# niclasborlin/dbat

Measured on AMD Instinct MI355X. Metric: LM iterations/sec, higher is better.
Workload: dtype f64

## Files before the change

dbat_amd/_hip.py:

```python
from __future__ import annotations

import ctypes as C
import os
import sys

import numpy as np

_HERE = os.path.dirname(os.path.abspath(__file__))
LIB_PATH = os.path.join(_HERE, 'libdbat_hip.so')
if os.environ.get('DBAT_AMD_LIB') == 'prof':
    LIB_PATH = os.path.join(_HERE, 'libdbat_hip_prof.so')
elif os.environ.get('DBAT_AMD_LIB', '').endswith('.so'):
    LIB_PATH = os.environ['DBAT_AMD_LIB']
if LIB_PATH != os.path.join(_HERE, 'libdbat_hip.so'):
    sys.stderr.write('[dbat_amd] DBAT_AMD_LIB: loading %s instead of the product library\n' % LIB_PATH)

ABI_VERSION = 5
DAMP = {'none': 0, 'gm': 0, 'gna': 1, 'lm': 2, 'lmp': 3}

OK, EINVAL, EUNSUPPORTED, EDEVICE, ENOMEM = 0, -101, -102, -103, -104


class DbatHipUnavailable(RuntimeError):
    pass
# ... 25 lines not shown
        ('device', C.c_int32), ('shard_rank', C.c_int32), ('shard_count', C.c_int32),
    ]


class Options(C.Structure):
    _fields_ = [
        ('damping', C.c_int32), ('max_iter', C.c_int32), ('conv_tol', C.c_double),
        ('abs_term', C.c_int32), ('singular_test', C.c_int32), ('store_trace', C.c_int32),
        ('mu', C.c_double), ('alpha_min', C.c_double), ('lambda0', C.c_double),
        ('lambda_min', C.c_double), ('rho_bad', C.c_double), ('rho_good', C.c_double),
        ('delta0', C.c_double),
        ('term_fun', C.c_void_p), ('term_user', C.c_void_p), ('veto_fun', C.c_void_p), ('veto_user', C.c_void_p),
        ('trace_fun', C.c_void_p), ('trace_user', C.c_void_p),
    ]


TERM_FN = C.CFUNCTYPE(C.c_int32, C.c_void_p, _dp, _dp, C.c_int64)
VETO_FN = C.CFUNCTYPE(C.c_int32, C.c_void_p, _dp, C.c_int64)
TRACE_FN = C.CFUNCTYPE(None, C.c_void_p, C.c_int32, C.c_int32, C.c_double, C.c_double, C.c_int32, C.c_double)


def trace_text(damping, n, res, damp, step, rho):
    from fractions import Fraction
    if damping == DAMP['gna']:
        if damp != damp:
            return 'Gauss-Newton-Armijo: iteration %d, residual norm=%.2g' % (n, res)
        return 'Gauss-Newton-Armijo: iteration %d, residual norm=%.2g, last alpha=%s' % (n, res, Fraction(damp).limit_denominator(1 << 40))
    if damping == DAMP['lm']:
        if damp != damp:
            return 'Levenberg-Marquardt: iteration %d, residual norm=%.2g' % (n, res)
        return 'Levenberg-Marquardt: iteration %d, residual norm=%.2g, lambda=%.2g' % (n, res, damp)
    if damping == DAMP['lmp']:
        return 'Levenberg-Marquardt-Powell: iteration %d, residual norm=%.2g, delta=%.2g, step=%s, rho=%.1f' % (
            n, res, damp, ('GN', 'IP', 'CP')[step] if 0 <= step < 3 else '?', rho)
    return 'Gauss-Markov: iteration %d, residual norm=%.2g' % (n, res)


class Result(C.Structure):
    _fields_ = [
        ('code', C.c_int32), ('iters', C.c_int32), ('n_res', C.c_int32), ('n_damp', C.c_int32),
        ('n_trace', C.c_int32), ('sigma0', C.c_double), ('time_s', C.c_double),
        ('n_residual_evals', C.c_int32), ('n_linearizations', C.c_int32), ('n_solves', C.c_int32),
        ('n_trace_only', C.c_int32), ('stage_s', C.c_double * 5),
    ]


LOSS = {'huber': 0, 'cauchy': 1}
SCALE = {'apriori': 0, 'mad': 1}
ROBUST_MAX_OUTER = 64


class RobustOptions(C.Structure):
    _fields_ = [
        ('loss', C.c_int32), ('k', C.c_double), ('scale', C.c_int32), ('max_outer', C.c_int32),
        ('weight_tol', C.c_double),
    ]


class PairOptions(C.Structure):
    _fields_ = [('max_iter', C.c_int32), ('conv_tol', C.c_double), ('min_angle', C.c_double)]


class RobustResult(C.Structure):
    _fields_ = [
        ('outer', C.c_int32), ('converged', C.c_int32), ('inner_iters', C.c_int32 * ROBUST_MAX_OUTER),
        ('scale', C.c_double * ROBUST_MAX_OUTER), ('max_change', C.c_double), ('reweight_s', C.c_double),
    ]


ALLREDUCE_FN = C.CFUNCTYPE(C.c_int, C.c_void_p, C.c_void_p, C.c_int64, C.c_void_p)

class DepthStats(C.Structure):
    _fields_ = [('n_behind', C.c_int64), ('min_depth', C.c_double), ('argmin_column', C.c_int64)]


class VetoStats(C.Structure):
    _fields_ = [('tested', C.c_int64), ('rejected', C.c_int64), ('n_behind', C.c_int64), ('min_depth', C.c_double)]


_H = C.c_void_p
SYMBOLS = {
    'dbat_hip_last_error': (C.c_char_p, []),
    'dbat_hip_abi_version': (C.c_int, []),
    'dbat_hip_default_options': (C.c_int, [C.c_int32, C.POINTER(Options)]),
    'dbat_hip_plan': (C.c_int, [C.POINTER(Problem)] + [C.POINTER(C.c_int64)] * 7),
    'dbat_hip_plan_structural_rank_ok': (C.c_int, [C.POINTER(Problem), C.POINTER(C.c_int32)]),
    'dbat_hip_plan_point_owner': (C.c_int, [C.POINTER(Problem), _ip]),
    'dbat_hip_plan_serialize': (C.c_int, [C.POINTER(Problem), _dp]),
    'dbat_hip_plan_layout_stats': (C.c_int, [C.POINTER(Problem), C.POINTER(C.c_int64)]),
    'dbat_hip_plan_domain_map': (C.c_int, [C.POINTER(Problem), _ip, C.POINTER(C.c_int32)]),
    'dbat_hip_create': (C.c_int, [C.POINTER(Problem), C.POINTER(_H)]),
    'dbat_hip_destroy': (None, [_H]),
    'dbat_hip_num_params': (C.c_int64, [_H]),
    'dbat_hip_num_residuals': (C.c_int64, [_H]),
    'dbat_hip_serialize': (C.c_int, [_H, _dp]),
    'dbat_hip_deserialize': (C.c_int, [_H, _dp, _dp, _dp, _dp]),
    'dbat_hip_structural_rank_ok': (C.c_int, [_H, C.POINTER(C.c_int32)]),
    'dbat_hip_residual': (C.c_int, [_H, _dp, _dp, _dp]),
    'dbat_hip_jacobian_blocks': (C.c_int, [_H, _dp, _dp, _dp, _dp]),
    'dbat_hip_jacobian_sample': (C.c_int, [_H, _dp, C.c_int64, C.POINTER(C.c_int64), _dp, _dp, _dp, _dp]),
    'dbat_hip_linearize_solve': (C.c_int, [_H, _dp, C.c_double, C.c_int32, _dp, _dp]),
    'dbat_hip_jacobian_csc': (C.c_int, [_H, _dp, C.c_int32, C.POINTER(C.c_int64), C.POINTER(C.c_int64), C.POINTER(C.c_int64), _dp]),
    'dbat_hip_gradient': (C.c_int, [_H, _dp]),
    'dbat_hip_colnorms': (C.c_int, [_H, _dp]),
    'dbat_hip_jtimes_sqnorm': (C.c_int, [_H, _dp, _dp]),
    'dbat_hip_jtimes': (C.c_int, [_H, _dp, _dp]),
    'dbat_hip_solve': (C.c_int, [_H, C.POINTER(Options), _dp, C.POINTER(Result), _dp, _dp, _dp, _dp]),
    'dbat_hip_final_residuals': (C.c_int, [_H, _dp, _dp]),
    'dbat_hip_comm_unique_id': (C.c_int, [_bp]),
    'dbat_hip_comm_init': (C.c_int, [_H, _bp]),
    'dbat_hip_comm_allreduce_host': (C.c_int, [_H, _dp, C.c_int64, C.c_int32]),
    'dbat_hip_set_deterministic': (C.c_int, [_H, C.c_int32]),
    'dbat_hip_set_allreduce': (C.c_int, [_H, ALLREDUCE_FN, C.c_void_p]),
    'dbat_hip_owned_mask': (C.c_int, [_H, _bp]),
    'dbat_hip_forwintersect': (C.c_int, [_H, _dp, _bp, _dp]),
    'dbat_hip_resect': (C.c_int, [C.c_int32, C.c_int32, C.POINTER(C.c_int64), _dp, _dp, C.POINTER(C.c_int64), _ip, _dp, _dp]),
    'dbat_hip_rigidalign': (C.c_int, [C.c_int32, C.c_int64, _dp, _dp, _bp, C.c_int32, _dp, _dp, _dp]),
    'dbat_hip_multixform': (C.c_int, [C.c_int32, _dp, C.c_int64, C.c_int32, _dp, C.c_int64, _dp, _bp]),
    'dbat_hip_essmat5': (C.c_int, [C.c_int32, C.c_int32, C.POINTER(C.c_int64), _dp, _dp, _dp, _ip]),
    'dbat_hip_relorient': (C.c_int, [C.c_int32, C.c_int32, C.POINTER(C.c_int64), _dp, _dp, C.POINTER(C.c_int64), _ip, _dp,
                                     C.c_int32, _dp, _dp, _ip, _bp, _bp, _dp]),
    'dbat_hip_default_pair_options': (C.c_int, [C.POINTER(PairOptions)]),
    'dbat_hip_pairadjust': (C.c_int, [C.c_int32, C.c_int32, C.POINTER(C.c_int64), _dp, _dp, _bp, _dp, _dp, C.c_int32,
                                      C.POINTER(PairOptions), _dp, _dp, _bp, _dp, _ip, _dp, _dp]),
    'dbat_hip_bench_step': (C.c_int, [_H, C.c_double, C.c_int32, _dp]),
    'dbat_hip_structure_key': (C.c_int, [C.POINTER(Problem), C.POINTER(C.c_uint64)]),
    'dbat_hip_handle_key': (C.c_int, [_H, C.POINTER(C.c_uint64)]),
    'dbat_hip_set_values': (C.c_int, [_H, C.POINTER(Problem)]),
    'dbat_hip_set_x': (C.c_int, [_H, _dp]),
    'dbat_hip_info': (C.c_int, [_H, C.POINTER(C.c_int64)]),
    'dbat_hip_build_kernel_name': (C.c_int, [_H, C.c_char_p, C.c_int32]),
    'dbat_hip_chol_stats': (C.c_int, [_H, C.POINTER(C.c_int64)]),
    'dbat_hip_posterior_cov': (C.c_int, [_H, _dp, C.c_double, _dp, _dp, _dp, _dp]),
    'dbat_hip_redundancy': (C.c_int, [_H, _dp, _dp, _dp]),
    'dbat_hip_ray_angles': (C.c_int, [_H, _dp, _dp, _dp, _ip, _ip]),
    'dbat_hip_debug_ray_angles_host': (C.c_int, [C.POINTER(Problem), _dp, _dp]),
    'dbat_hip_point_depths': (C.c_int, [_H, _dp, C.c_double, _dp, _dp, C.POINTER(DepthStats)]),
    'dbat_hip_set_chirality': (C.c_int, [_H, C.c_int32, C.c_double]),
    'dbat_hip_chirality_stats': (C.c_int, [_H, C.POINTER(VetoStats)]),
    'dbat_hip_coverage': (C.c_int, [_H, _dp, _dp, _dp, _lp, _dp, _lp, _lp]),
    'dbat_hip_residual_stats': (C.c_int, [_H, _dp, _lp, _dp, _lp, _dp, _dp, _dp, _lp]),
    'dbat_hip_quality_hull_cap': (C.c_int32, []),
    'dbat_hip_debug_coverage_host': (C.c_int, [C.POINTER(Problem), _dp, _dp, _dp, _lp, _dp, _lp, _lp]),
    'dbat_hip_default_robust_options': (C.c_int, [C.c_int32, C.POINTER(RobustOptions)]),
    'dbat_hip_robust_weights': (C.c_int, [_H, _dp, C.POINTER(RobustOptions), _dp, _dp, _dp]),
    'dbat_hip_set_obs_weights': (C.c_int, [_H, _dp]),
    'dbat_hip_solve_robust': (C.c_int, [_H, C.POINTER(Options), C.POINTER(RobustOptions), _dp, C.POINTER(Result),
                                        _dp, _dp, _dp, _dp, C.POINTER(RobustResult), _dp]),
}
DEBUG_SYMBOLS = {
    'dbat_hip_debug_plan_digest': (C.c_int, [C.POINTER(Problem), C.POINTER(C.c_uint64), C.c_int32, C.c_char_p, C.c_int32]),
    'dbat_hip_debug_heavy_plan_selftest': (C.c_int, [C.POINTER(Problem), _dp]),
    'dbat_hip_debug_batch_stats': (C.c_int, [C.POINTER(Problem), C.POINTER(C.c_int64)]),
    'dbat_hip_debug_model_eval_host': (C.c_int, [C.c_int32, C.c_int32, C.c_int32, _dp, _dp, C.c_double,
                                                 _dp, _dp, _dp, _dp, _dp, _dp]),
    'dbat_hip_debug_ray_angles_ms': (C.c_int, [_H, _dp, C.POINTER(C.c_int64)]),
    'dbat_hip_debug_quality_ms': (C.c_int, [_H, _dp]),
    'dbat_hip_debug_point_depths_ms': (C.c_int, [_H, _dp]),
    'dbat_hip_debug_chirality_pass_ms': (C.c_int, [_H, _dp, C.c_int32, _dp]),
    'dbat_hip_debug_align_ms': (C.c_int, [_dp]),
    'dbat_hip_debug_align_timing': (C.c_int, [C.c_int32]),
    'dbat_hip_debug_relorient_ms': (C.c_int, [_dp]),
    'dbat_hip_debug_relorient_timing': (C.c_int, [C.c_int32]),
    'dbat_hip_debug_pairadjust_ms': (C.c_int, [_dp]),
    'dbat_hip_debug_pairadjust_timing': (C.c_int, [C.c_int32]),
}

_lib = None


def load():
    global _lib
    if _lib is not None:
        return _lib
    if not os.path.exists(LIB_PATH):
        raise DbatHipUnavailable(
            '%s not built: run `python -c "import __graft_entry__ as g; g.build()"` or '
            '`make -C dbat_amd/csrc` (needs hipcc).  There is no CPU fallback.' % LIB_PATH)
    try:
        try:
            import torch
        except Exception:
            pass
        lib = C.CDLL(LIB_PATH)
    except OSError as e:
        raise DbatHipUnavailable('cannot load %s: %s' % (LIB_PATH, e)) from e
    for name, (res, args) in {**SYMBOLS, **DEBUG_SYMBOLS}.items():
        try:
            fn = getattr(lib, name)
        except AttributeError as e:
            raise DbatHipUnavailable('%s does not export %s' % (LIB_PATH, name)) from e
        fn.restype = res
        fn.argtypes = args
    if lib.dbat_hip_abi_version() != ABI_VERSION:
        raise DbatHipUnavailable('ABI version mismatch')
    _lib = lib
    return lib


UNIQUE_ID_BYTES = 128


def comm_unique_id():
    buf = (C.c_uint8 * UNIQUE_ID_BYTES)()
    check(load().dbat_hip_comm_unique_id(buf))
    return bytes(buf)


def last_error():
    return load().dbat_hip_last_error().decode('utf-8', 'replace')


def check(rc):
    if rc != 0:
        raise DbatHipError(rc, last_error())


def dptr(a):
    return a.ctypes.data_as(_dp) if a is not None else None


def _flat(a, dtype):
    a = np.asarray(a)
    if a.dtype != dtype:
        a = a.astype(dtype)
    if a.ndim <= 1:
        return np.ascontiguousarray(a)
    if a.flags.f_contiguous:
        return a.reshape(-1, order='F')
    return a.flatten('F')


def _f64(a):
    return _flat(a, np.float64)


def _u8(a):
    a = np.asarray(a)
    if a.dtype != np.bool_:
        a = a.astype(bool)
    return _flat(a, np.bool_).view(np.uint8)


def _i32(a):
    return _flat(a, np.int32)


def problem_from_struct(s, device=0, shard_rank=0, shard_count=1):
    nc, npnt, no = s.EO.val.shape[1], s.OP.val.shape[1], s.IP.val.shape[1]
    dm = np.unique(s.IO.model.distModel)
    if dm.size != 1:
        raise ValueError('Mixed lens distortion models not implemented.')
    model = int(dm[0])
    if model == 1:
        if np.any(np.asarray(s.IO.val)[3:5] != 0) or np.any(np.asarray(s.bundle.est.IO)[3:5]):
            raise ValueError('lens distortion model 1 has no aspect/skew')
        model = 2
    if npnt >= 2 ** 31 or nc >= 2 ** 31:
        raise ValueError('too many points/images for int32 indices')
    keep = dict(
        ip_cam=_i32(s.IP.cam), ip_pt=_i32(s.IP.pt), ip_val=_f64(s.IP.val), ip_std=_f64(s.IP.std),
        IO_val=_f64(s.IO.val), px_size=_f64(s.IO.sensor.pxSize), EO_val=_f64(s.EO.val[:6]),
        OP_val=_f64(s.OP.val),
        est_IO=_u8(s.bundle.est.IO), est_EO=_u8(s.bundle.est.EO[:6]), est_OP=_u8(s.bundle.est.OP),
        IO_block=_i32(s.IO.struct.block), EO_block=_i32(s.EO.struct.block[:6]),
    )
    for nm in ('IO', 'EO', 'OP'):
        pr = getattr(s.prior, nm)
        rows = slice(0, 6) if nm == 'EO' else slice(None)
        use = np.asarray(pr.use)[rows]
        keep['prior_%s_use' % nm] = _u8(use)
        if use.any():
            keep['prior_%s_val' % nm] = _f64(np.nan_to_num(np.asarray(pr.val, float)[rows]))
            keep['prior_%s_std' % nm] = _f64(np.nan_to_num(np.asarray(pr.std, float)[rows], nan=1.0))
        else:
            keep['prior_%s_val' % nm] = _f64(np.asarray(pr.val, float)[rows])
            keep['prior_%s_std' % nm] = _f64(np.asarray(pr.std, float)[rows])
    p = Problem()
    p.abi_version = ABI_VERSION
    p.n_images, p.n_points, p.n_obs = nc, npnt, no
    p.dist_model, p.nK, p.nP = model, int(s.IO.model.nK), int(s.IO.model.nP)
    for k, v in keep.items():
        ptr_t = dict(Problem._fields_)[k]
        setattr(p, k, v.ctypes.data_as(ptr_t))
    p.device, p.shard_rank, p.shard_count = int(device), int(shard_rank), int(shard_count)
    return p, keep


class Handle:

    def __init__(self, s, device=0, shard_rank=0, shard_count=1, _problem=None):
        self.lib = load()
        self.prob, self._keep = _problem if _problem is not None else problem_from_struct(s, device, shard_rank, shard_count)
        h = _H()
        check(self.lib.dbat_hip_create(C.byref(self.prob), C.byref(h)))
        self.h = h
        self.n = int(self.lib.dbat_hip_num_params(h))
        self.m = int(self.lib.dbat_hip_num_residuals(h))
        self._cb = None

    def close(self):
        if getattr(self, 'h', None):
            self.lib.dbat_hip_destroy(self.h)
            self.h = None

    __del__ = close
# ... 493 lines not shown
    return dict(E=E[:9 * n].reshape(n, 9), P2=P2[:12 * n].reshape(n, 4, 3).transpose(0, 2, 1), stats=st[:8 * n].reshape(n, 8),
                inlier=inl[:total].astype(bool), in_front=fr[:total].astype(bool), X=X[:3 * total].reshape(3, total, order='F'))


def cams_from_e(e, x1, x2, front_dir, device=0):
    lib = load()
    x1, x2 = np.asarray(x1, float), np.asarray(x2, float)
    if x1.ndim != 2 or x1.shape[0] != 2 or x1.shape != x2.shape:
        raise ValueError('camsfrome: the points must be 2-by-n')
    n = x1.shape[1]
    ps = np.array([0, n], np.int64)
    a, b, E, t2 = _f64(x1), _f64(x2), np.ascontiguousarray(np.asarray(e, float).reshape(9)).copy(), np.ones(1)
    P2, st = np.zeros(12), np.zeros(8, np.int32)
    inl, fr, X = np.zeros(max(n, 1), np.uint8), np.zeros(max(n, 1), np.uint8), np.zeros(3 * max(n, 1))
    check(lib.dbat_hip_relorient(int(device), 1, ps.ctypes.data_as(C.POINTER(C.c_int64)), dptr(a), dptr(b), None, None, dptr(t2),
                                 int(front_dir), dptr(E), dptr(P2), st.ctypes.data_as(_ip), inl.ctypes.data_as(_bp),
                                 fr.ctypes.data_as(_bp), dptr(X)))
    return dict(P2=P2.reshape(4, 3).T.copy(), X=X[:3 * n].reshape(3, n, order='F'), in_front=fr[:n].astype(bool), sp=st[4:8].copy())


def relorient_timing(on=True):
    check(load().dbat_hip_debug_relorient_timing(int(bool(on))))


def relorient_ms():
    ms = np.zeros(3)
    check(load().dbat_hip_debug_relorient_ms(dptr(ms)))
    return dict(solve=float(ms[0]), score=float(ms[1]), cams=float(ms[2]))


PAIR_CODES = ('converged', 'max_iter', 'no_step', 'singular', 'too_few')


def pairadjust(pt_start, x1, x2, P2, X, use=None, w1=None, w2=None, front_dir=-1, max_iter=20, conv_tol=1e-6, min_angle=0.0,
               residuals=False, device=0):
    lib = load()
    ps = np.ascontiguousarray(pt_start, np.int64)
    n = len(ps) - 1
    x1, x2, X = np.asarray(x1, float), np.asarray(x2, float), np.asarray(X, float)
    P2 = np.asarray(P2, float).reshape(-1, 3, 4)
    if n < 0 or x1.ndim != 2 or x1.shape[0] != 2 or x1.shape != x2.shape or x1.shape[1] != ps[-1] or X.shape != (3, x1.shape[1]) \
            or P2.shape[0] != n:
        raise ValueError('pairadjust: x1 and x2 must be 2-by-total, X 3-by-total, total the end of the last range, and P2 one 3-by-4 per pair')
    total = x1.shape[1]
    a, b = _f64(x1), _f64(x2)
    wt = [None if w is None else _f64(np.broadcast_to(np.asarray(w, float), (2, total))) for w in (w1, w2)]
    u = None if use is None else np.ascontiguousarray(np.broadcast_to(np.asarray(use, bool), (total,))).view(np.uint8)
    P = np.ascontiguousarray(P2.transpose(0, 2, 1)).reshape(-1).copy()
    P = np.concatenate([P, np.zeros(12)]) if n == 0 else P
    Xf = X.flatten('F')
    Xf = np.zeros(3) if total == 0 else Xf
    used, ds, ist, Q = np.zeros(max(total, 1), np.uint8), np.zeros(4 * max(n, 1)), np.zeros(4 * max(n, 1), np.int32), np.zeros(36 * max(n, 1))
    res = np.zeros(4 * max(total, 1)) if residuals else None
    opt = PairOptions(int(max_iter), float(conv_tol), float(min_angle))
    check(lib.dbat_hip_pairadjust(int(device), n, ps.ctypes.data_as(C.POINTER(C.c_int64)), dptr(a), dptr(b),
                                  None if u is None else u.ctypes.data_as(_bp), dptr(wt[0]), dptr(wt[1]), int(front_dir), C.byref(opt),
                                  dptr(P), dptr(Xf), used.ctypes.data_as(_bp), dptr(ds), ist.ctypes.data_as(_ip), dptr(Q), dptr(res)))
    ds, ist = ds[:4 * n].reshape(n, 4), ist[:4 * n].reshape(n, 4)
    return dict(P2=P[:12 * n].reshape(n, 4, 3).transpose(0, 2, 1), X=Xf[:3 * total].reshape(3, total, order='F'), used=used[:total].astype(bool),
                f0=ds[:, 0].copy(), f=ds[:, 1].copy(), sigma0=ds[:, 2].copy(), lam=ds[:, 3].copy(), code=ist[:, 0].copy(),
                iters=ist[:, 1].copy(), trials=ist[:, 2].copy(), n_used=ist[:, 3].copy(), Q=Q[:36 * n].reshape(n, 6, 6).transpose(0, 2, 1),
                res=None if res is None else res[:4 * total].reshape(total, 2, 2).transpose(1, 2, 0))


def pairadjust_timing(on=True):
    check(load().dbat_hip_debug_pairadjust_timing(int(bool(on))))


def pairadjust_ms():
    ms = np.zeros(1)
    check(load().dbat_hip_debug_pairadjust_ms(dptr(ms)))
    return float(ms[0])


def rigidalign(X, Y, scale=False, use=None, resid=False, device=0):
    lib = load()
    X, Y = np.asarray(X, float), np.asarray(Y, float)
    if X.ndim != 2 or X.shape[0] != 3 or X.shape != Y.shape:
        raise ValueError('rigidalign: X and Y must both be 3-by-n')
    n = X.shape[1]
    Xf, Yf = _f64(X), _f64(Y)
    u = None
    if use is not None:
        u = np.ascontiguousarray(np.asarray(use, bool).ravel()).view(np.uint8)
        if u.shape[0] != n:
            raise ValueError('rigidalign: use must have one entry per column')
    T, st = np.zeros(16), np.zeros(4)
    r = np.empty(3 * n) if resid else None
    check(lib.dbat_hip_rigidalign(int(device), n, dptr(Xf), dptr(Yf), None if u is None else u.ctypes.data_as(_bp),
                                  int(bool(scale)), dptr(T), dptr(st), dptr(r)))
    return (T.reshape(4, 4, order='F'), dict(alpha=float(st[0]), rms=float(st[1]), used=int(st[2]), sv_ratio=float(st[3])),
            None if r is None else r.reshape(3, n, order='F'))


def multixform(EO, OP, T, device=0):
    lib = load()
    EO, OP, T = np.asarray(EO, float), np.asarray(OP, float), np.asarray(T, float)
    if T.shape != (4, 4):
        raise ValueError('multixform: T must be 4-by-4')
    EO = np.zeros((6, 0)) if EO.size == 0 else EO
    OP = np.zeros((3, 0)) if OP.size == 0 else OP
    if EO.ndim != 2 or OP.ndim != 2 or (OP.size and OP.shape[0] != 3):
        raise ValueError('multixform: EO must be 6-by-M (or more rows), OP 3-by-N')
    nc, npnt = (EO.shape[1] if EO.size else 0), (OP.shape[1] if OP.size else 0)
    rows = EO.shape[0] if nc else 6
    eo, op = np.array(EO, float, order='F'), np.array(OP, float, order='F')
    fail = np.zeros(max(nc, 1), np.uint8)
    check(lib.dbat_hip_multixform(int(device), dptr(_f64(T)), nc, int(rows), dptr(eo.reshape(-1, order='F')) if nc else None,
                                  npnt, dptr(op.reshape(-1, order='F')) if npnt else None, fail.ctypes.data_as(_bp)))
    return eo, op, fail[:nc].astype(bool)


def align_timing(on=True):
    check(load().dbat_hip_debug_align_timing(int(bool(on))))


def align_ms():
    ms = np.zeros(5)
    check(load().dbat_hip_debug_align_ms(dptr(ms)))
    return dict(centroid=float(ms[0]), cross=float(ms[1]), resid=float(ms[2]), points=float(ms[3]), cams=float(ms[4]))


def plan_layout_stats(s, shard_rank=0, shard_count=1):
    lib = load()
    p, keep = problem_from_struct(s, 0, shard_rank, shard_count)
    a = (C.c_int64 * 16)()
    check(lib.dbat_hip_plan_layout_stats(C.byref(p), a))
    v = [int(x) for x in a]
    return dict(n_tiles=v[0], n_batches=v[1], n_batches_tiled=v[2], n_groups=v[3], n_group_points=v[4], n_chunks=v[5],
                chunks_by_length={'1-8': v[6], '9-16': v[7], '17-32': v[8], '33-64': v[9]}, chunks_multi_round=v[10],
                k_max=v[11], rows_max=v[12], build_sig=bool(v[13]), backsub_sig=bool(v[14]), heavy_tasks=v[15])


def plan_digest(s, shard_rank=0, shard_count=1):
    lib = load()
    p, keep = problem_from_struct(s, 0, shard_rank, shard_count)
    out = (C.c_uint64 * 96)()
    names = C.create_string_buffer(4096)
    n = lib.dbat_hip_debug_plan_digest(C.byref(p), out, 96, names, 4096)
    if n < 0:
        check(n)
    return dict(zip(names.value.decode().split(','), [int(v) for v in out[:n]]))


def heavy_plan_selftest(s, shard_rank=0, shard_count=1):
    lib = load()
    p, keep = problem_from_struct(s, 0, shard_rank, shard_count)
    out = np.zeros(8)
    check(lib.dbat_hip_debug_heavy_plan_selftest(C.byref(p), dptr(out)))
    return dict(on=bool(out[0]), points=int(out[1]), row_groups=int(out[2]), tasks=int(out[3]), ksteps=int(out[4]),
                max_diff=float(out[5]), max_abs=float(out[6]), entries=int(out[7]))


def batch_stats(s, shard_rank=0, shard_count=1):
    lib = load()
    p, keep = problem_from_struct(s, 0, shard_rank, shard_count)
    a = (C.c_int64 * 16)()
    check(lib.dbat_hip_debug_batch_stats(C.byref(p), a))
    v = [int(x) for x in a]
    part = lambda q: dict(max_points=v[q], max_obs=v[q + 1], closed_by_cap=v[q + 2], max_tile_batches=v[q + 3])
    return dict(tiled=part(0), untiled=part(4), BT=v[8], PMAX=v[9], tile_bmax=v[10], n_batches_tiled=v[11],
                n_batches_untiled=v[12])


def plan_domain_map(s, shard_count):
    lib = load()
    p, keep = problem_from_struct(s, 0, 0, shard_count)
    owner = np.full(s.EO.val.shape[1], -1, np.int32)
    sub = C.c_int32(0)
    check(lib.dbat_hip_plan_domain_map(C.byref(p), owner.ctypes.data_as(_ip), C.byref(sub)))
    return owner, bool(sub.value)


def plan_serialize(s):
    lib = load()
    p, keep = problem_from_struct(s)
    x0 = np.empty(plan(s)['n'])
    check(lib.dbat_hip_plan_serialize(C.byref(p), dptr(x0)))
    return x0


def debug_model_eval_host(model, nK, nP, EO6, IO, px, Q, uv):
    lib = load()
    R = 5 + nK + nP
    r, A, B, Cc = np.zeros(2), np.zeros(12), np.zeros(6), np.zeros(2 * R)
    a = [np.ascontiguousarray(v, float) for v in (EO6, IO, Q, uv)]
    check(lib.dbat_hip_debug_model_eval_host(model, nK, nP, dptr(a[0]), dptr(a[1]), float(px),
                                             dptr(a[2]), dptr(a[3]), dptr(r), dptr(A), dptr(B), dptr(Cc)))
    return r, A.reshape(6, 2).T, B.reshape(3, 2).T, Cc.reshape(R, 2).T


def _coverage_call(fn, nc, no):
    lo, hi = np.zeros(2 * max(nc, 1)), np.zeros(2 * max(nc, 1))
    rad, area = np.zeros(max(nc, 1)), np.zeros(max(nc, 1))
    rip, hs, hip = np.zeros(max(nc, 1), np.int64), np.zeros(nc + 1, np.int64), np.zeros(max(no, 1), np.int64)
    lp = lambda a: a.ctypes.data_as(_lp)
    check(fn(dptr(lo), dptr(hi), dptr(rad), lp(rip), dptr(area), lp(hs), lp(hip)))
    return dict(lo=lo[:2 * nc].reshape(2, nc, order='F'), hi=hi[:2 * nc].reshape(2, nc, order='F'), rad_max=rad[:nc],
                rad_ip=rip[:nc], hull_area=area[:nc], hull=[hip[hs[c]:hs[c + 1]].copy() for c in range(nc)])


def quality_hull_cap():
    return int(load().dbat_hip_quality_hull_cap())


def debug_coverage_host(s):
    lib = load()
    p, keep = problem_from_struct(s)
    return _coverage_call(lambda *a: lib.dbat_hip_debug_coverage_host(C.byref(p), *a), int(p.n_images), int(p.n_obs))


def debug_ray_angles_host(s):
    lib = load()
    p, keep = problem_from_struct(s)
    op, cam = np.zeros(max(int(p.n_points), 1)), np.zeros(max(int(p.n_images), 1))
    check(lib.dbat_hip_debug_ray_angles_host(C.byref(p), dptr(op), dptr(cam)))
    return op[:int(p.n_points)], cam[:int(p.n_images)]
```

dbat_amd/csrc/chol_df.hpp:

```cpp
#pragma once
#include "env.hpp"
#include <cstdio>
#include <functional>
#include <queue>

#include "chol.hpp"
#include "nd.hpp"

namespace dbat {

constexpr int DF_LD = 65;
constexpr int DF_SPIN_CAP = 1 << 22;

struct DfTask { int i, k; };
struct DfJob { int i, k, jlo, jhi, part, np, mode, p; };

__device__ __forceinline__ double ld_coh(const double *p) {
    return __hip_atomic_load(p, __ATOMIC_RELAXED, __HIP_MEMORY_SCOPE_AGENT);
}
__device__ __forceinline__ void st_coh(double *p, double v) {
    __hip_atomic_store(p, v, __ATOMIC_RELAXED, __HIP_MEMORY_SCOPE_AGENT);
}

typedef double df_d2 __attribute__((ext_vector_type(2)));
// ... 923 lines not shown
    __shared__ double smem[2 * 64 * LD];
    double *Pm = smem, *Qm = smem + 64 * LD;
    const int tx = threadIdx.x & 63, ty = threadIdx.x >> 6;
    const SiTask tk = tasks[blockIdx.x];
    double *T = tiles + toff[(int64_t)tk.i * nT + tk.k];
    si_load_T<LD>(linv_all + (size_t)tk.k * 4096, Pm, tx, ty);
    si_load<LD>(T, Qm, tx, ty);
    __syncthreads();
    chol_d4 acc[4] = {{0, 0, 0, 0}, {0, 0, 0, 0}, {0, 0, 0, 0}, {0, 0, 0, 0}};
    mfma_tile64<LD>(Pm, Qm, ty, tx, acc);
#pragma unroll
    for (int rt = 0; rt < 4; ++rt)
#pragma unroll
        for (int e = 0; e < 4; ++e) T[(16 * ty + (tx >> 4) + 4 * e) * 64 + 16 * rt + (tx & 15)] = acc[rt][e];
}
__global__ __launch_bounds__(256) void k_selinv_off(double *__restrict__ Z, const double *__restrict__ M, const int64_t *__restrict__ toff,
                                                    int nT, const int *__restrict__ bk_ptr, const int *__restrict__ bk_idx,
                                                    const SiTask *__restrict__ tasks) {
    constexpr int LD = DF_LD;
    __shared__ double smem[2 * 64 * LD];
    double *Pm = smem, *Qm = smem + 64 * LD;
    const int tx = threadIdx.x & 63, ty = threadIdx.x >> 6;
    const SiTask tk = tasks[blockIdx.x];
    const int i = tk.i, k = tk.k;
    chol_d4 acc[4] = {{0, 0, 0, 0}, {0, 0, 0, 0}, {0, 0, 0, 0}, {0, 0, 0, 0}};
    for (int e = bk_ptr[k]; e < bk_ptr[k + 1]; ++e) {
        const int j = bk_idx[e];
        __syncthreads();
        si_load_T<LD>(M + toff[(int64_t)j * nT + k], Pm, tx, ty);
        if (i >= j) si_load<LD>(Z + toff[(int64_t)i * nT + j], Qm, tx, ty);
        else si_load_T<LD>(Z + toff[(int64_t)j * nT + i], Qm, tx, ty);
        __syncthreads();
        mfma_tile64<LD>(Pm, Qm, ty, tx, acc);
    }
    double *T = Z + toff[(int64_t)i * nT + k];
#pragma unroll
    for (int rt = 0; rt < 4; ++rt)
#pragma unroll
        for (int e = 0; e < 4; ++e) T[(16 * ty + (tx >> 4) + 4 * e) * 64 + 16 * rt + (tx & 15)] = -acc[rt][e];
}
__global__ __launch_bounds__(256) void k_selinv_diag(double *__restrict__ Z, const double *__restrict__ M, const int64_t *__restrict__ toff,
                                                     int nT, const int *__restrict__ bk_ptr, const int *__restrict__ bk_idx,
                                                     const double *__restrict__ linv_all, const int *__restrict__ cols) {
    constexpr int LD = DF_LD;
    __shared__ double smem[2 * 64 * LD];
    double *Pm = smem, *Qm = smem + 64 * LD;
    const int tx = threadIdx.x & 63, ty = threadIdx.x >> 6;
    const int k = cols[blockIdx.x];
    chol_d4 acc[4] = {{0, 0, 0, 0}, {0, 0, 0, 0}, {0, 0, 0, 0}, {0, 0, 0, 0}};
    si_load_T<LD>(linv_all + (size_t)k * 4096, Pm, tx, ty);
    __syncthreads();
    mfma_tile64<LD>(Pm, Pm, ty, tx, acc);
    for (int e = bk_ptr[k]; e < bk_ptr[k + 1]; ++e) {
        const int j = bk_idx[e];
        __syncthreads();
        si_load_T<LD>(Z + toff[(int64_t)j * nT + k], Pm, tx, ty);
        si_load_T<LD>(M + toff[(int64_t)j * nT + k], Qm, tx, ty, -1.0);
        __syncthreads();
        mfma_tile64<LD>(Pm, Qm, ty, tx, acc);
    }
    double *T = Z + toff[(int64_t)k * nT + k];
#pragma unroll
    for (int rt = 0; rt < 4; ++rt)
#pragma unroll
        for (int e = 0; e < 4; ++e) T[(16 * ty + (tx >> 4) + 4 * e) * 64 + 16 * rt + (tx & 15)] = acc[rt][e];
}

struct DataflowChol {
    int n = 0, n_nat = 0, nT = 0, W = 0, ntasks = 0, ntiles = 0, epoch = 0, grid = 512;
    bool permuted = false;
    bool reset_done = false;
    bool reset_args(int *&ctl, unsigned long long *&q, int &nq) const {
        if (!permuted || !d_ctl || !d_qperm) return false;
        ctl = d_ctl; q = reinterpret_cast<unsigned long long *>(d_qperm); nq = nT * CHOL_NB;
        return true;
    }
    long long n_products = 0;
    int *d_flags = nullptr, *d_ctl = nullptr, *d_bk_ptr = nullptr, *d_bk_idx = nullptr, *d_iperm = nullptr;
    int64_t *d_toff = nullptr;
    uint64_t *d_rowbits = nullptr;
    DfJob *d_tasks = nullptr, *d_tasksB = nullptr;
    int ntasksB = 0, nbk = 0;
    int *d_bk_list = nullptr;
    uint64_t *d_rowbits_top = nullptr;
    bool two_phase = false;
    int64_t top_tile0 = 0, n_top_tiles = 0;
    std::vector<double> sim_critical_us, sim_schedule_us;
    std::vector<DfJob> h_tasksB;
    DfTask *d_tile_ij = nullptr;
    int nparts = 0;
    bool env_l2 = false;
    int env_df_ablate = 0;
    bool use_chain = false;
    int nchain = 0, nchainB = 0, chain_wg = 0, chain_wgB = 0;
    int *d_chain_cols = nullptr, *d_chain_colsB = nullptr, *d_chain_par = nullptr, *d_chain_bits = nullptr, *d_chain_bitsB = nullptr, *d_chain_pos = nullptr;
    double *d_parts = nullptr;
    double *d_tiles = nullptr, *d_qperm = nullptr;
    double *d_ztiles = nullptr;
    SiTask *d_si_m = nullptr, *d_si_off = nullptr;
    int *d_si_diag = nullptr, *d_perm = nullptr;
    int n_si_m = 0;
    std::vector<int> si_off_ptr, si_diag_ptr;
    std::vector<uint64_t> h_rowbits;
    long long *d_trace = nullptr;
    std::vector<DfJob> h_tasks;
    std::vector<int> perm;
    size_t linv_doubles() const { return (size_t)std::max(nT, 1) * CHOL_NB * CHOL_NB; }

    void release() {
        void *ps[] = {d_flags, d_ctl, d_bk_ptr, d_bk_idx, d_iperm, d_toff, d_rowbits, d_tasks, d_tile_ij, d_tiles, d_qperm, d_parts,
                      d_tasksB, d_bk_list, d_rowbits_top, d_chain_cols, d_chain_colsB, d_chain_par, d_chain_bits, d_chain_bitsB, d_chain_pos,
                      d_ztiles, d_si_m, d_si_off, d_si_diag, d_perm};
        for (void *p : ps) if (p) (void)hipFree(p);
        d_flags = d_ctl = d_bk_ptr = d_bk_idx = d_iperm = nullptr; d_toff = nullptr; d_rowbits = nullptr;
        d_tasks = nullptr; d_tile_ij = nullptr; d_tiles = d_qperm = d_parts = nullptr;
        d_tasksB = nullptr; d_bk_list = nullptr; d_rowbits_top = nullptr;
        d_chain_cols = d_chain_colsB = d_chain_par = d_chain_bits = d_chain_bitsB = d_chain_pos = nullptr;
        d_ztiles = nullptr; d_si_m = d_si_off = nullptr; d_si_diag = d_perm = nullptr; n_si_m = 0;
        si_off_ptr.clear(); si_diag_ptr.clear();
    }
    void dump_trace(hipStream_t stream, const char *path) const {
        if (!d_trace) return;
        std::vector<long long> h((size_t)(ntasks + 3 * nT) * 16);
        (void)hipStreamSynchronize(stream);
        (void)hipMemcpy(h.data(), d_trace, h.size() * sizeof(long long), hipMemcpyDeviceToHost);
        FILE *f = fopen(path, "w");
        if (!f) return;
        for (int t = 0; t < ntasks + nT; ++t) {
            const int i = t < ntasks ? (h_tasks[t].np < 0 ? -(h_tasks[t].i + 2) : h_tasks[t].i) : -1, k = t < ntasks ? h_tasks[t].k : nT - 1 - (t - ntasks);
            fprintf(f, "%d,%d,%d", t, i, k);
            for (int q = 0; q < 16; ++q) fprintf(f, ",%lld", h[(size_t)t * 16 + q]);
            fprintf(f, ",%d,%d,%d\n", t < ntasks ? h_tasks[t].jlo : 0, t < ntasks ? (h_tasks[t].np < 0 ? h_tasks[t].jhi : h_tasks[t].k) : 0,
                    t < ntasks ? h_tasks[t].mode : 0);
        }
        for (int k = 0; k < nT && use_chain; ++k) {
            fprintf(f, "%d,-3,%d", ntasks + nT + k, k);
            for (int q = 0; q < 16; ++q) fprintf(f, ",%lld", h[(size_t)(ntasks + nT + k) * 16 + q]);
            fprintf(f, ",0,0,0\n");
        }
        for (int k = 0; k < nT && use_chain; ++k) {
            fprintf(f, "%d,-4,%d", ntasks + 2 * nT + k, k);
            for (int q = 0; q < 16; ++q) fprintf(f, ",%lld", h[(size_t)(ntasks + 2 * nT + k) * 16 + q]);
            fprintf(f, ",0,0,0\n");
        }
        fclose(f);
    }
    template <class T>
    static bool up(T *&dst, const std::vector<T> &v) {
        if (hipMalloc((void **)&dst, std::max<size_t>(v.size(), 1) * sizeof(T)) != hipSuccess) return false;
        if (!v.empty()) (void)hipMemcpy(dst, v.data(), v.size() * sizeof(T), hipMemcpyHostToDevice);
        return true;
    }
    struct JobList { std::vector<DfJob> jobs; std::vector<int> dptr, dep, own, sumjob, presum, bits, par; };
    void build_jobs(int phase, const std::vector<uint64_t> &rowbits, const std::vector<int> &col_owner, int rank, JobList &L) {
        auto has = [&](int i, int k) { return (rowbits[(size_t)i * W + (k >> 6)] >> (k & 63)) & 1ull; };
        const int split_min = std::max(env_int("DBAT_HIP_DF_SPLIT", 96), 2);
        const int chunk = std::max(env_int("DBAT_HIP_DF_CHUNK", 32), 1);
        const bool merge = permuted;
        auto top = [&](int k) { return phase != 0 && col_owner[k] < 0; };
        auto mine = [&](int k) { return phase == 0 || col_owner[k] == rank; };
        int dom_lo = nT, dom_hi = 0;
        if (phase == 1) for (int k = 0; k < nT; ++k) if (col_owner[k] == rank) { dom_lo = std::min(dom_lo, k); dom_hi = k + 1; }
        if (dom_hi <= dom_lo) dom_lo = dom_hi = 0;
        L.jobs.clear(); L.dptr.assign(1, 0); L.dep.clear();
        L.own.assign((size_t)(nT + 1) * nT, -1); L.sumjob.assign(nT, -1);
        L.presum.assign(nT, -1); L.bits.assign(nT, 0); L.par.assign(nT, -1);
        const bool chain = use_chain && merge;
        auto inphase = [&](int c) { return c < nT && (phase == 0 || (phase == 1 ? col_owner[c] == rank : col_owner[c] < 0)); };
        std::vector<int> js;
        for (int k = 0; k < nT; ++k) {
            auto emit = [&](int i, int mode, int par, int jhi_owner) {
                n_products += (long long)js.size();
                const int nj = (int)js.size();
                const int nch = nj > split_min ? (nj + chunk - 1) / chunk : 1;
                auto push_products = [&](int q0, int q1) {
                    for (int q = q0; q < q1; ++q) { L.dep.push_back(L.own[(size_t)k * nT + js[q]]); L.dep.push_back(i != k ? L.own[(size_t)i * nT + js[q]] : -1); }
                    L.dptr.push_back((int)L.dep.size());
                };
                for (int c = 0; c + 1 < nch; ++c) {
                    L.jobs.push_back(DfJob{i, k, js[chunk * c], js[chunk * (c + 1)], nparts + c, -1, 0, -1});
                    push_products(chunk * c, chunk * (c + 1));
                }
                const int me = (int)L.jobs.size();
                L.jobs.push_back(DfJob{i, k, nch > 1 ? js[chunk * (nch - 1)] : (nj ? js[0] : jhi_owner), jhi_owner, nparts, nch - 1, mode, i == k ? par : -1});
                push_products(chunk * (nch - 1), nj);
                nparts += nch - 1;
                return me;
            };
            if (phase == 1 && top(k)) {
                for (int i = k; i <= nT; ++i) {
                    if (!has(i, k)) continue;
                    js.clear();
                    for (int j = dom_lo; j < std::min(dom_hi, k); ++j) if (has(i, j) && has(k, j)) js.push_back(j);
                    emit(i, rank == 0 ? 4 : 12, -1, std::min(dom_hi, k));
                }
                continue;
            }
            if (phase == 1 ? !mine(k) : (phase == 2 && !top(k))) continue;
            auto products = [&](int i) {
                js.clear();
                for (int j = 0; j < k; ++j) if (has(i, j) && has(k, j) && (phase != 2 || top(j))) js.push_back(j);
            };
            int par = -1;
            if (merge) for (int i = k + 1; i <= nT && par < 0; ++i) if (has(i, k)) par = i;
            if (par >= 0) { products(par); L.sumjob[k] = emit(par, 1, -1, k); }
            products(k);
            L.par[k] = par;
            if (chain) {
                const bool cont = k > 0 && (L.bits[k - 1] & 2) != 0;
                if (cont) js.pop_back();
                L.presum[k] = emit(k, 16, -1, cont ? k - 1 : k);
                js.clear();
                L.bits[k] = (cont ? 1 : 0) | ((par == k + 1 && k + 1 < nT && inphase(k + 1)) ? 2 : 0);
            }
            L.own[(size_t)k * nT + k] = emit(k, par >= 0 ? 2 : 0, par, k);
            if (par >= 0) L.own[(size_t)par * nT + k] = L.own[(size_t)k * nT + k];
            for (int i = k + 1; i <= nT; ++i)
                if (has(i, k) && i != par) { products(i); L.own[(size_t)i * nT + k] = emit(i, 0, -1, k); }
        }
    }
    void order_jobs(JobList &L, const char *what) {
        std::vector<DfJob> &jobs = L.jobs;
        const std::vector<int> &dptr = L.dptr, &dep = L.dep, &own = L.own, &sumjob = L.sumjob;
        const int nt = (int)jobs.size();
        if (nt == 0) return;
        auto is_helper = [&](int t) { return jobs[t].np < 0; };
        auto is_share = [&](int t) { return (jobs[t].mode & 4) != 0; };
        auto is_diag = [&](int t) { return jobs[t].np >= 0 && jobs[t].i == jobs[t].k && !is_share(t) && jobs[t].mode != 16; };
        auto nprod_of = [&](int t) { return (dptr[t + 1] - dptr[t]) / 2; };
        auto for_deps = [&](int t, const std::function<void(int)> &f) {
            for (int q = dptr[t]; q < dptr[t + 1]; ++q) if (dep[q] >= 0) f(dep[q]);
            if (!is_helper(t)) {
                for (int h = 1; h <= jobs[t].np; ++h) f(t - h);
                if (jobs[t].mode == 0 && jobs[t].i != jobs[t].k) f(own[(size_t)jobs[t].k * nT + jobs[t].k]);
                if (jobs[t].mode == 2) f(sumjob[jobs[t].k]);
                if (is_diag(t) && L.presum[jobs[t].k] >= 0) {
                    f(L.presum[jobs[t].k]);
                    if (L.bits[jobs[t].k] & 1) f(own[(size_t)(jobs[t].k - 1) * nT + jobs[t].k - 1]);
                }
            }
        };
        const double c_prod = 2.5, c_diag = 13.5, c_off = 4.5, c_hop = 2.0, c_add = 1.5, c_help = 2.0;
        auto tail_of = [&](int t) { return is_helper(t) || is_share(t) || jobs[t].mode == 1 || jobs[t].mode == 16 ? c_help : (is_diag(t) ? c_diag + (jobs[t].mode == 2 ? 2.5 : 0.0) : c_off); };
        std::vector<double> est(nt, 0.0), fin(nt, 0.0);
        for (int t = 0; t < nt; ++t) {
            double e = 0.0;
            for_deps(t, [&](int d) { e = std::max(e, fin[d]); });
            est[t] = e;
            fin[t] = e + c_hop + (nprod_of(t) ? c_prod : 0.0) + tail_of(t);
        }
        std::vector<double> blev(nt, 0.0);
        for (int t = nt - 1; t >= 0; --t) {
            blev[t] += c_hop + c_prod + tail_of(t);
            for_deps(t, [&](int d) { blev[d] = std::max(blev[d], blev[t]); });
        }
        const int workers = std::max(1, std::min(grid, 256));
        auto simulate = [&](const std::vector<int> &ord) {
            std::vector<double> done(nt, 0.0);
            std::priority_queue<double, std::vector<double>, std::greater<double>> freeat;
            for (int w = 0; w < workers; ++w) freeat.push(0.0);
            double last = 0.0;
            for (int t : ord) {
                double tc = freeat.top(); freeat.pop();
                for (int q = dptr[t]; q + 1 < dptr[t + 1]; q += 2) {
                    double av = done[dep[q]];
                    if (dep[q + 1] >= 0) av = std::max(av, done[dep[q + 1]]);
                    tc = std::max(tc, av + c_hop) + c_prod;
                }
                if (!is_helper(t)) {
                    for (int h = jobs[t].np; h >= 1; --h) tc = std::max(tc, done[t - h] + c_hop) + c_add;
                    if (jobs[t].mode == 0 && jobs[t].i != jobs[t].k) tc = std::max(tc, done[own[(size_t)jobs[t].k * nT + jobs[t].k]] + c_hop);
                    if (jobs[t].mode == 2) tc = std::max(tc, done[sumjob[jobs[t].k]] + c_hop - c_diag);
                    if (is_diag(t) && L.presum[jobs[t].k] >= 0) {
                        tc = std::max(tc, done[L.presum[jobs[t].k]] + c_hop);
                        if (L.bits[jobs[t].k] & 1) tc = std::max(tc, done[own[(size_t)(jobs[t].k - 1) * nT + jobs[t].k - 1]]);
                    }
                }
                tc += tail_of(t);
                done[t] = tc; last = std::max(last, tc);
                freeat.push(tc);
            }
            return last;
        };
        std::vector<int> indeg0(nt, 0), sptr(nt + 1, 0), succ;
        for (int t = 0; t < nt; ++t) for_deps(t, [&](int d) { ++indeg0[t]; ++sptr[d + 1]; });
        for (int t = 0; t < nt; ++t) sptr[t + 1] += sptr[t];
        succ.resize(sptr[nt]);
        {
            std::vector<int> fill(sptr.begin(), sptr.end() - 1);
            for (int t = 0; t < nt; ++t) for_deps(t, [&](int d) { succ[fill[d]++] = t; });
        }
        auto kahn = [&](const std::vector<double> &key) {
            std::vector<int> ord(nt), indeg(indeg0);
            typedef std::pair<double, int> KI;
            std::priority_queue<KI, std::vector<KI>, std::greater<KI>> pq;
            for (int t = 0; t < nt; ++t) if (!indeg[t]) pq.push(KI(key[t], t));
            size_t n_out = 0;
            while (!pq.empty()) {
                const int t = pq.top().second; pq.pop();
                ord[n_out++] = t;
                for (int q = sptr[t]; q < sptr[t + 1]; ++q) if (--indeg[succ[q]] == 0) pq.push(KI(key[succ[q]], succ[q]));
            }
            return ord;
        };
        const double betas[] = {0.0, 0.25, 0.5, 1.0, 2.0, 4.0, 1e6};
        const int ncand = (int)(sizeof(betas) / sizeof(betas[0])) + 1;
        std::vector<int> best_ord;
        double tbest = 1e300;
        int best = -1;
        std::vector<double> key(nt), tcs(ncand);
        const int forced = env_int("DBAT_HIP_DF_ORDER", -1);
        for (int c = 0; c < ncand; ++c) {
            if (c + 1 < ncand) for (int t = 0; t < nt; ++t) key[t] = est[t] - betas[c] * blev[t];
            else for (int t = 0; t < nt; ++t) key[t] = est[t] - c_prod * nprod_of(t);
            std::vector<int> ord = kahn(key);
            tcs[c] = simulate(ord);
            if (forced == c || (forced < 0 && tcs[c] < tbest)) { tbest = tcs[c]; best = c; best_ord.swap(ord); }
        }
        double cp = 0.0;
        for (int t = 0; t < nt; ++t) cp = std::max(cp, fin[t]);
        sim_critical_us.push_back(cp); sim_schedule_us.push_back(tbest);
        if (env_on("DBAT_HIP_PLAN_STATS")) {
            fprintf(stderr, "[chol %s] %d tasks, critical path %.0f us; simulated with %d workgroups, key = earliest start - beta x bottom level:",
                    what, nt, cp, workers);
            for (int c = 0; c + 1 < ncand; ++c) fprintf(stderr, " beta %g: %.0f us,", betas[c], tcs[c]);
            fprintf(stderr, " earliest start - own work: %.0f us -> candidate %d\n", tcs[ncand - 1], best);
        }
        std::vector<DfJob> sorted(nt);
        for (int t = 0; t < nt; ++t) sorted[t] = jobs[best_ord[t]];
        jobs.swap(sorted);
    }
    bool finish_setup(const std::vector<uint64_t> &rowbits, const std::vector<int64_t> &toff,
                      const std::vector<int> &col_owner = std::vector<int>(), int rank = 0) {
        auto has = [&](int i, int k) { return (rowbits[(size_t)i * W + (k >> 6)] >> (k & 63)) & 1ull; };
        if (const char *g = env_get("DBAT_HIP_DF_GRID")) grid = std::min(std::max(atoi(g), 1), 4096);
        nparts = 0; n_products = 0;
        two_phase = !col_owner.empty();
        h_rowbits = rowbits;
        use_chain = permuted && env_int("DBAT_HIP_DF_CHAIN", 1) != 0;
        if (use_chain && !two_phase && !env_get("DBAT_HIP_DF_CHAIN")) {
            long long nprod = 0;
            int longest = 0, cur = 0;
            for (int k = 0; k < nT; ++k) {
                int par = -1;
                for (int i = k; i <= nT; ++i) {
                    if (!has(i, k)) continue;
                    if (i > k && par < 0) par = i;
                    for (int w = 0; w < W; ++w) {
                        uint64_t m = rowbits[(size_t)i * W + w] & rowbits[(size_t)k * W + w];
                        if (w == (k >> 6)) m &= (1ull << (k & 63)) - 1;
                        else if (w > (k >> 6)) m = 0;
                        nprod += __builtin_popcountll(m);
                    }
                }
                cur = (k > 0 && cur > 0) ? cur : 1;
                longest = std::max(longest, cur);
                cur = par == k + 1 ? cur + 1 : 0;
            }
            const double t_products = (double)nprod * 2.6 / std::min(grid, 256), t_chain = longest * 17.0;
            use_chain = t_products < 0.6 * t_chain;
            if (env_on("DBAT_HIP_PLAN_STATS"))
                fprintf(stderr, "[chol] %lld tile products (%.0f us over the workgroups), longest chain %d links (%.0f us): chain role %s\n",
                        nprod, t_products, longest, t_chain, use_chain ? "on" : "off");
        }
        auto split_chain = [&](JobList &L, std::vector<DfJob> &tasks, std::vector<int> &cols) {
            tasks.clear(); cols.clear();
            for (const DfJob &j : L.jobs) {
                if (use_chain && j.np >= 0 && j.i == j.k && (j.mode == 0 || j.mode == 2)) cols.push_back(j.k);
                else tasks.push_back(j);
            }
        };
        auto chain_width = [&](const std::vector<int> &cols, const std::vector<int> &bits) {
            int runs = 0;
            for (int k : cols) runs += !(bits[k] & 1);
            return std::max(1, std::min(runs, env_int("DBAT_HIP_DF_CHAIN_WG", 32)));
        };
        std::vector<int> colsA, colsB;
        sim_critical_us.clear(); sim_schedule_us.clear();
        JobList L;
        std::vector<int> bkl;
        std::vector<uint64_t> rowbits_top;
        if (!two_phase) {
            build_jobs(0, rowbits, col_owner, rank, L);
            order_jobs(L, "all");
            split_chain(L, h_tasks, colsA); ntasks = (int)h_tasks.size();
            for (int j = nT - 1; j >= 0; --j) bkl.push_back(j);
        } else {
            build_jobs(1, rowbits, col_owner, rank, L);
            order_jobs(L, "domain");
            split_chain(L, h_tasks, colsA); ntasks = (int)h_tasks.size();
            JobList B;
            build_jobs(2, rowbits, col_owner, rank, B);
            order_jobs(B, "top");
            split_chain(B, h_tasksB, colsB); ntasksB = (int)h_tasksB.size();
            if (!up(d_tasksB, h_tasksB)) return false;
            if (use_chain) {
                for (int k = 0; k < nT; ++k) if (B.par[k] >= 0) L.par[k] = B.par[k];
                nchainB = (int)colsB.size(); chain_wgB = chain_width(colsB, B.bits);
                if (!up(d_chain_colsB, colsB) || !up(d_chain_bitsB, B.bits)) return false;
            }
            for (int j = nT - 1; j >= 0; --j) if (col_owner[j] < 0) bkl.push_back(j);
            for (int j = nT - 1; j >= 0; --j) if (col_owner[j] == rank) bkl.push_back(j);
            rowbits_top = rowbits;
            for (int i = 0; i <= nT; ++i)
                for (int k = 0; k < nT; ++k)
                    if (col_owner[k] >= 0) rowbits_top[(size_t)i * W + (k >> 6)] &= ~(1ull << (k & 63));
            if (!up(d_rowbits_top, rowbits_top)) return false;
        }
        nbk = (int)bkl.size();
        if (use_chain) {
            nchain = (int)colsA.size(); chain_wg = chain_width(colsA, L.bits);
            std::vector<int> pos(nT, 0);
            for (size_t q = 0; q < colsA.size(); ++q) pos[colsA[q]] = (int)q;
            for (size_t q = 0; q < colsB.size(); ++q) pos[colsB[q]] = (int)q;
            if (!up(d_chain_cols, colsA) || !up(d_chain_bits, L.bits) || !up(d_chain_par, L.par) || !up(d_chain_pos, pos)) return false;
            if (env_on("DBAT_HIP_PLAN_STATS")) {
                int runs = 0, longest = 0, cur = 0;
                for (int k = 0; k < nT; ++k) { if (L.bits[k] & 1) ++cur; else { cur = 1; } longest = std::max(longest, cur); }
                for (int k : colsA) runs += !(L.bits[k] & 1);
                fprintf(stderr, "[chol] chain role: %d diagonal tiles in %d chains (longest %d), %d workgroups%s\n", nchain, runs, longest, chain_wg,
                        two_phase ? " (domain)" : "");
            }
        }
        if (env_on("DBAT_HIP_DF_TRACE") && !two_phase && hipMalloc(&d_trace, (size_t)(ntasks + 3 * nT) * 16 * sizeof(long long)) != hipSuccess) d_trace = nullptr;
        std::vector<int> bptr(nT + 1, 0), bidx;
        for (int j = 0; j < nT; ++j) {
            for (int i = nT - 1; i > j; --i)
                if (has(i, j)) bidx.push_back(i);
            bptr[j + 1] = (int)bidx.size();
        }
        if (!up(d_tasks, h_tasks) || !up(d_bk_ptr, bptr) || !up(d_bk_idx, bidx) || !up(d_rowbits, rowbits) || !up(d_toff, toff) || !up(d_bk_list, bkl))
            return false;
        if (hipMalloc(&d_flags, ((size_t)(nT + 1) * nT + (size_t)nparts + 4 * (size_t)nT) * sizeof(int)) != hipSuccess) return false;
        if (nparts > 0 && hipMalloc(&d_parts, (size_t)nparts * 4096 * sizeof(double)) != hipSuccess) return false;
        if (hipMalloc(&d_ctl, 8 * sizeof(int)) != hipSuccess) return false;
        (void)hipMemset(d_flags, 0, ((size_t)(nT + 1) * nT + (size_t)nparts + 4 * (size_t)nT) * sizeof(int));
        (void)hipMemset(d_ctl, 0, 8 * sizeof(int));
        env_l2 = env_int("DBAT_HIP_DF_L2", 0) != 0;
        env_df_ablate = 2 * (env_int("DBAT_HIP_DF_ABLATE", 0) & 3);
        epoch = 0;
        return true;
    }
    bool setup_inplace(const CholEnvelope &env, int64_t lda) {
        release();
        permuted = false; perm.clear();
        n = n_nat = env.n; nT = (n + CHOL_NB - 1) / CHOL_NB; W = (nT + 64) / 64;
        std::vector<uint64_t> rb((size_t)(nT + 1) * W, 0);
        std::vector<int64_t> toff((size_t)(nT + 1) * nT, -1);
        for (int i = 0; i <= nT; ++i) {
            const int kf = i < nT ? env.panel_first[i] / CHOL_NB : 0;
            for (int k = kf; k <= std::min(i, nT - 1); ++k) {
                rb[(size_t)i * W + (k >> 6)] |= 1ull << (k & 63);
                toff[(size_t)i * nT + k] = (int64_t)CHOL_NB * k * lda + (i == nT ? (int64_t)n : (int64_t)CHOL_NB * i);
            }
        }
        return finish_setup(rb, toff);
    }
    bool setup_permuted(int nc, int nio, const uint64_t *adj, int adj_words, const NdTree &nd, int rank) {
        release();
        permuted = true;
        n_nat = 6 * nc + nio;
        const std::vector<int> &order = nd.order, &block_end = nd.block_end;
        std::vector<int> rowpos(nc);
        int off = 0;
        {
            const bool pad_all = env_on("DBAT_HIP_ND_PAD_ALL");
            size_t b = 0; int q0 = 0;
            for (int q = 0; q < nc; ++q) {
                if (q == q0) {
                    const int sep_rows = 6 * (block_end[b] - q0), used = off % CHOL_NB;
                    const bool saves = used > 0 && (used + sep_rows + CHOL_NB - 1) / CHOL_NB < 1 + (sep_rows + CHOL_NB - 1) / CHOL_NB;
                    const int join_small = env_int("DBAT_HIP_ND_JOIN_SMALL", 2 * CHOL_NB);
                    const bool joins = !pad_all && (saves || (used > 0 && sep_rows <= join_small)) && b > 0 && b < nd.block_sep.size() && nd.block_sep[b] &&
                                       nd.block_owner[b] == nd.block_owner[b - 1];
                    if (!joins) off = (off + CHOL_NB - 1) / CHOL_NB * CHOL_NB;
                }
                rowpos[order[q]] = off; off += 6;
                while (b < block_end.size() && block_end[b] <= q + 1) { q0 = q + 1; ++b; }
            }
        }
        const int io0 = nio > 0 ? (off + CHOL_NB - 1) / CHOL_NB * CHOL_NB : off;
        n = (io0 + nio + CHOL_NB - 1) / CHOL_NB * CHOL_NB;
        nT = n / CHOL_NB; W = (nT + 64) / 64;
        perm.assign(n_nat, 0);
        std::vector<int> iperm((size_t)n, -1);
        for (int c = 0; c < nc; ++c)
            for (int a = 0; a < 6; ++a) perm[6 * c + a] = rowpos[c] + a;
        for (int u = 0; u < nio; ++u) perm[6 * nc + u] = io0 + u;
        for (int z = 0; z < n_nat; ++z) iperm[perm[z]] = z;
        auto pos6 = [&](int c) { return rowpos[c]; };
        std::vector<uint64_t> rb((size_t)(nT + 1) * W, 0);
        auto setbit = [&](int i, int k) { rb[(size_t)i * W + (k >> 6)] |= 1ull << (k & 63); };
        for (int a = 0; a < nc; ++a) {
            const int ta0 = pos6(a) / CHOL_NB, ta1 = (pos6(a) + 5) / CHOL_NB;
            for (int w = 0; w < adj_words; ++w) {
                uint64_t m = adj[(size_t)a * adj_words + w];
                while (m) {
                    const int b = 64 * w + __builtin_ctzll(m);
                    m &= m - 1;
                    if (b >= nc) break;
                    const int tb0 = pos6(b) / CHOL_NB, tb1 = (pos6(b) + 5) / CHOL_NB;
                    for (int ti = ta0; ti <= ta1; ++ti)
                        for (int tj = tb0; tj <= tb1; ++tj) setbit(std::max(ti, tj), std::min(ti, tj));
                }
            }
            for (int ti = ta0; ti <= ta1; ++ti) for (int tj = ta0; tj <= ti; ++tj) setbit(ti, tj);
        }
        for (int i = 0; i < nT; ++i) setbit(i, i);
        for (int i = io0 / CHOL_NB; i < nT && nio > 0; ++i) for (int k = 0; k <= i; ++k) setbit(i, k);
        for (int k = 0; k < nT; ++k) setbit(nT, k);
        {
            std::vector<int> rows;
            for (int k = 0; k < nT; ++k) {
                rows.clear();
                for (int i = k + 1; i <= nT; ++i) if ((rb[(size_t)i * W + (k >> 6)] >> (k & 63)) & 1ull) rows.push_back(i);
                for (size_t a = 0; a < rows.size(); ++a)
                    for (size_t b = 0; b <= a; ++b)
                        if (rows[b] < nT) setbit(rows[a], rows[b]);
            }
        }
        std::vector<int> col_owner;
        if (nd.nparts > 1) {
            col_owner.assign(nT, -1);
            size_t b = 0;
            for (int q = 0; q < nc; ++q) {
                while (b < block_end.size() && block_end[b] <= q) ++b;
                const int ow = b < nd.block_owner.size() ? nd.block_owner[b] : -1;
                for (int t = rowpos[order[q]] / CHOL_NB; t <= (rowpos[order[q]] + 5) / CHOL_NB; ++t) col_owner[t] = ow;
            }
        }
        std::vector<int64_t> toff((size_t)(nT + 1) * nT, -1);
        std::vector<DfTask> tile_ij;
        for (int pass = 0; pass < 2; ++pass) {
            if (pass == 1) top_tile0 = (int64_t)tile_ij.size();
            for (int k = 0; k < nT; ++k) {
                if ((!col_owner.empty() && col_owner[k] < 0) != (pass == 1)) continue;
                for (int i = k; i <= nT; ++i)
                    if ((rb[(size_t)i * W + (k >> 6)] >> (k & 63)) & 1ull) {
                        toff[(size_t)i * nT + k] = (int64_t)tile_ij.size() * 4096;
                        tile_ij.push_back(DfTask{i, k});
                    }
            }
        }
        ntiles = (int)tile_ij.size();
        n_top_tiles = ntiles - top_tile0;
        if (!up(d_tile_ij, tile_ij) || !up(d_iperm, iperm)) return false;
        if (hipMalloc(&d_tiles, (size_t)ntiles * 4096 * sizeof(double)) != hipSuccess) return false;
        (void)hipMemset(d_tiles, 0, (size_t)ntiles * 4096 * sizeof(double));
        if (hipMalloc(&d_qperm, (size_t)nT * CHOL_NB * sizeof(double)) != hipSuccess) return false;
        if (env_on("DBAT_HIP_PLAN_STATS"))
            fprintf(stderr, "[chol] order %d (%d with block padding, %zu blocks), %d tile rows, %d tiles (%.1f MB), dense lower triangle would be %d tiles\n",
                    n_nat, n, block_end.size(), nT, ntiles, ntiles * 32768.0 / 1e6, nT * (nT + 1) / 2 + nT);
        if (env_on("DBAT_HIP_PLAN_STATS")) {
            fprintf(stderr, "[chol] cameras per block, last (root separator) first:");
            for (size_t b = block_end.size(); b-- > 0 && block_end.size() - b <= 24;)
                fprintf(stderr, " %d", block_end[b] - (b ? block_end[b - 1] : 0));
            fprintf(stderr, "\n");
        }
        if (env_on("DBAT_HIP_PLAN_STATS") && !col_owner.empty()) {
            int ntop = 0, nmine = 0;
            for (int k = 0; k < nT; ++k) { ntop += col_owner[k] < 0; nmine += col_owner[k] == rank; }
            fprintf(stderr, "[chol] rank %d of %d: %d tile columns in its domain, %d top columns, %lld top tiles (%.1f MB summed over the ranks per factorisation)\n",
                    rank, nd.nparts, nmine, ntop, (long long)n_top_tiles, n_top_tiles * 32768.0 / 1e6);
        }
        return finish_setup(rb, toff, col_owner, rank);
    }
    bool selinv_supported() const { return permuted && !two_phase; }
    bool selected_inverse(hipStream_t stream, const double *linv_work) {
        if (!d_ztiles) {
            auto has = [&](int i, int k) { return (h_rowbits[(size_t)i * W + (k >> 6)] >> (k & 63)) & 1ull; };
            std::vector<SiTask> mt, off;
            std::vector<int> level(nT, 0), diag;
            int nlev = 0;
            for (int k = nT - 1; k >= 0; --k) {
                int lv = 0;
                for (int i = k + 1; i < nT; ++i) if (has(i, k)) { lv = std::max(lv, level[i] + 1); mt.push_back(SiTask{i, k}); }
                level[k] = lv; nlev = std::max(nlev, lv + 1);
            }
            si_off_ptr.assign(nlev + 1, 0); si_diag_ptr.assign(nlev + 1, 0);
            for (int lv = 0; lv < nlev; ++lv) {
                for (int k = nT - 1; k >= 0; --k) {
                    if (level[k] != lv) continue;
                    diag.push_back(k);
                    for (int i = k + 1; i < nT; ++i) if (has(i, k)) off.push_back(SiTask{i, k});
                }
                si_off_ptr[lv + 1] = (int)off.size(); si_diag_ptr[lv + 1] = (int)diag.size();
            }
            n_si_m = (int)mt.size();
            if (!up(d_si_m, mt) || !up(d_si_off, off) || !up(d_si_diag, diag) || !up(d_perm, perm)) return false;
            if (hipMalloc(&d_ztiles, (size_t)ntiles * 4096 * sizeof(double)) != hipSuccess) { d_ztiles = nullptr; return false; }
        }
        if (n_si_m > 0)
            hipLaunchKernelGGL(k_selinv_m, dim3(n_si_m), dim3(256), 0, stream, d_tiles, d_toff, nT, linv_work, d_si_m);
        for (size_t lv = 0; lv + 1 < si_off_ptr.size(); ++lv) {
            const int no = si_off_ptr[lv + 1] - si_off_ptr[lv], nd = si_diag_ptr[lv + 1] - si_diag_ptr[lv];
            if (no > 0)
                hipLaunchKernelGGL(k_selinv_off, dim3(no), dim3(256), 0, stream, d_ztiles, (const double *)d_tiles, d_toff, nT, d_bk_ptr,
                                   d_bk_idx, d_si_off + si_off_ptr[lv]);
            if (nd > 0)
                hipLaunchKernelGGL(k_selinv_diag, dim3(nd), dim3(256), 0, stream, d_ztiles, (const double *)d_tiles, d_toff, nT, d_bk_ptr,
                                   d_bk_idx, linv_work, d_si_diag + si_diag_ptr[lv]);
        }
        return true;
    }
    int selinv_levels() const { return (int)si_off_ptr.size() - 1; }
    void solve(hipStream_t stream, double *A, int64_t lda, double *q_out, double *linv_work, int *info_dev,
               double *ldiag = nullptr, const double *qscale = nullptr, double *dz_out = nullptr) {
        if (d_trace) (void)hipMemsetAsync(d_trace, 0, (size_t)(ntasks + 3 * nT) * 16 * sizeof(long long), stream);
        ++epoch;
        DfView V;
        V.toff = d_toff; V.rowbits = d_rowbits; V.W = W; V.no_l2 = (env_l2 ? 0 : 1) | env_df_ablate;
        double *qflag;
        V.S = nullptr; V.ldS = lda; V.n_nat = n_nat;
        if (permuted) {
            if (!reset_done)
                hipLaunchKernelGGL(k_df_reset, dim3((nT * CHOL_NB + 255) / 256), dim3(256), 0, stream, info_dev, d_ctl,
                                   reinterpret_cast<unsigned long long *>(d_qperm), nT * CHOL_NB);
            reset_done = false;
            V.base = d_tiles; V.ld = 64; V.iperm = d_iperm; qflag = d_qperm; V.S = A;
        } else {
            (void)hipMemsetAsync(info_dev, 0, sizeof(int), stream);
            (void)hipMemsetAsync(d_ctl, 0, 8 * sizeof(int), stream);
            V.base = A; V.ld = lda; V.iperm = nullptr; qflag = q_out;
            (void)hipMemsetAsync(q_out, 0xFF, (size_t)n * sizeof(double), stream);
        }
        if (permuted && use_chain)
            hipLaunchKernelGGL(k_chol_df<true>, dim3(chain_grid(ntasks + nT, chain_wg)), dim3(256), 0, stream, V, n, nT, d_tasks, ntasks,
                               d_flags, d_ctl, epoch, linv_work, info_dev, d_trace, d_bk_ptr, d_bk_idx, qflag, q_out, ldiag,
                               qscale, dz_out, d_parts, nparts, d_bk_list, nbk, 0, chain_arg(0));
        else
            hipLaunchKernelGGL(k_chol_df<false>, dim3(std::min(grid, ntasks + nT)), dim3(256), 0, stream, V, n, nT, d_tasks, ntasks,
                               d_flags, d_ctl, epoch, linv_work, info_dev, d_trace, d_bk_ptr, d_bk_idx, qflag, q_out, ldiag,
                               qscale, dz_out, d_parts, nparts, d_bk_list, nbk, 0, DfChain{});
    }
    DfChain chain_arg(int which) const {
        DfChain C;
        int *dfl = d_flags + (size_t)(nT + 1) * nT + nparts + nT;
        C.cols = which ? d_chain_colsB : d_chain_cols; C.ncols = which ? nchainB : nchain;
        C.par = d_chain_par; C.bits = which ? d_chain_bitsB : d_chain_bits;
        C.dflags = dfl; C.claim = dfl + nT; C.giveup = dfl + 2 * nT; C.pos = d_chain_pos;
        C.nwg = which ? chain_wgB : chain_wg;
        C.ctr_slot = which ? 5 : 3; C.role_slot = which ? 6 : 4;
        C.trace_potf2 = env_int("DBAT_HIP_DF_TRACE_POTF2", 0);
        return C;
    }
    int chain_grid(int work, int wg) const { return std::max(std::min(grid, work + wg), wg + 1); }
    double *top_tiles() const { return d_tiles + top_tile0 * 4096; }
    int64_t top_tiles_count() const { return n_top_tiles * 4096; }
    void solve_domain(hipStream_t stream, double *A, int64_t lda, double *linv_work, int *info_dev, double *ldiag) {
        ++epoch;
        DfView V;
        V.toff = d_toff; V.rowbits = d_rowbits; V.W = W; V.no_l2 = (env_l2 ? 0 : 1) | env_df_ablate;
        V.ldS = lda; V.n_nat = n_nat; V.base = d_tiles; V.ld = 64; V.iperm = d_iperm; V.S = A;
        hipLaunchKernelGGL(k_df_reset, dim3((nT * CHOL_NB + 255) / 256), dim3(256), 0, stream, info_dev, d_ctl,
                           reinterpret_cast<unsigned long long *>(d_qperm), nT * CHOL_NB);
        if (ntasks > 0 && use_chain)
            hipLaunchKernelGGL(k_chol_df<true>, dim3(chain_grid(ntasks, chain_wg)), dim3(256), 0, stream, V, n, nT, d_tasks, ntasks,
                               d_flags, d_ctl, epoch, linv_work, info_dev, (long long *)nullptr, d_bk_ptr, d_bk_idx, (double *)nullptr,
                               (double *)nullptr, ldiag, (const double *)nullptr, (double *)nullptr, d_parts, nparts, d_bk_list, 0, 0, chain_arg(0));
        else if (ntasks > 0)
            hipLaunchKernelGGL(k_chol_df<false>, dim3(std::min(grid, ntasks)), dim3(256), 0, stream, V, n, nT, d_tasks, ntasks,
                               d_flags, d_ctl, epoch, linv_work, info_dev, (long long *)nullptr, d_bk_ptr, d_bk_idx, (double *)nullptr,
                               (double *)nullptr, ldiag, (const double *)nullptr, (double *)nullptr, d_parts, nparts, d_bk_list, 0, 0, DfChain{});
    }
    void solve_top(hipStream_t stream, int64_t lda, double *q_out, double *linv_work, int *info_dev, double *ldiag,
                   const double *qscale, double *dz_out) {
        DfView V;
        V.toff = d_toff; V.rowbits = d_rowbits_top; V.W = W; V.no_l2 = 1;
        V.ldS = lda; V.n_nat = n_nat; V.base = d_tiles; V.ld = 64; V.iperm = d_iperm; V.S = nullptr;
        if (use_chain)
            hipLaunchKernelGGL(k_chol_df<true>, dim3(chain_grid(ntasksB + nbk, chain_wgB)), dim3(256), 0, stream, V, n, nT, d_tasksB, ntasksB,
                               d_flags, d_ctl, epoch, linv_work, info_dev, (long long *)nullptr, d_bk_ptr, d_bk_idx, d_qperm, q_out, ldiag,
                               qscale, dz_out, d_parts, nparts, d_bk_list, nbk, 2, chain_arg(1));
        else
            hipLaunchKernelGGL(k_chol_df<false>, dim3(std::min(grid, ntasksB + nbk)), dim3(256), 0, stream, V, n, nT, d_tasksB, ntasksB,
                               d_flags, d_ctl, epoch, linv_work, info_dev, (long long *)nullptr, d_bk_ptr, d_bk_idx, d_qperm, q_out, ldiag,
                               qscale, dz_out, d_parts, nparts, d_bk_list, nbk, 2, DfChain{});
    }
};

}
```

dbat_amd/csrc/dbat_core.hip:

```cpp
#include <hip/hip_runtime.h>
#include <rocblas/rocblas.h>
#include <rocsolver/rocsolver.h>
#include <rccl/rccl.h>

#include <algorithm>
#include <chrono>
#include <cmath>
#include <cstdio>
#include <cstdlib>
#include <memory>
#include <string>
#include <thread>
#include <type_traits>
#include <utility>
#include <atomic>
#include <vector>

#include "../../include/dbat_hip.h"
#include "chol_df.hpp"
#include "kernels.hpp"
#include "cov.hpp"
#include "sig.hpp"
#include "heavy.hpp"
#include "plan.hpp"
#include "resect.hpp"
#include "robust.hpp"
#include "angles.hpp"
#include "depth.hpp"
#include "quality.hpp"
#include "align.hpp"
#include "relorient.hpp"
#include "pairadjust.hpp"

namespace dbat {

static thread_local std::string g_err;

struct DeviceError { std::string msg; };
struct UsageError { std::string msg; };

#define HIPCHK(expr)                                                                       \
    do {                                                                                   \
        hipError_t e_ = (expr);                                                            \
        if (e_ != hipSuccess)                                                              \
            throw DeviceError{std::string(#expr) + ": " + hipGetErrorString(e_)};          \
    } while (0)

template <auto K, class... A>
static void launch(dim3 grid, dim3 block, size_t lds, hipStream_t stream, A &&...args) {
    hipLaunchKernelGGL(K, grid, block, lds, stream, std::forward<A>(args)...);
    HIPCHK(hipGetLastError());
}

template <auto V, auto... Vs, class T, class F>
static inline void with_value(T v, F &&f) {
    if constexpr (sizeof...(Vs) == 0) f(std::integral_constant<decltype(V), V>{});
    else if (v == V) f(std::integral_constant<decltype(V), V>{});
    else with_value<Vs...>(v, f);
}

struct DeviceGuard {
    int prev = -1, dev = -1;
    explicit DeviceGuard(int device) : dev(device) {
        if (hipGetDevice(&prev) != hipSuccess) prev = -1;
        if (prev != dev) HIPCHK(hipSetDevice(dev));
    }
    ~DeviceGuard() { if (prev >= 0 && prev != dev) (void)hipSetDevice(prev); }
};

#define NCCLCHK(expr)                                                                      \
    do {                                                                                   \
        ncclResult_t r_ = (expr);                                                          \
        if (r_ != ncclSuccess)                                                             \
            throw DeviceError{std::string(#expr) + ": " + ncclGetErrorString(r_)};         \
    } while (0)

template <class T>
struct DevBuf {
    T *p = nullptr;
    size_t n = 0;
    void alloc(size_t count) {
        n = count;
        if (count) HIPCHK(hipMalloc((void **)&p, count * sizeof(T)));
    }
    void upload(const T *src, size_t count) {
        alloc(count);
        if (count) HIPCHK(hipMemcpy(p, src, count * sizeof(T), hipMemcpyHostToDevice));
    }
    template <class A>
    void upload(const std::vector<T, A> &v) { upload(v.data(), v.size()); }
    ~DevBuf() { if (p) (void)hipFree(p); }
};

static double event_ms(hipEvent_t a, hipEvent_t b) { float t = 0; HIPCHK(hipEventElapsedTime(&t, a, b)); return t; }
template <int N>
struct EventTimer {
    hipEvent_t ev[N + 1] = {};
    int n = 0;
    double ms[N] = {};
    ~EventTimer() { for (auto &e : ev) if (e) (void)hipEventDestroy(e); }
    void start(hipStream_t s) {
        if (!ev[0]) for (auto &e : ev) HIPCHK(hipEventCreate(&e));
        HIPCHK(hipEventRecord(ev[n = 0], s));
    }
    void lap(hipStream_t s) { if (ev[0]) HIPCHK(hipEventRecord(ev[++n], s)); }
    double read() { for (int i = 0; ev[0] && i < N; ++i) ms[i] = event_ms(ev[i], ev[i + 1]); return ms[0]; }
};

static inline int64_t cdiv(int64_t a, int64_t b) { return (a + b - 1) / b; }
static inline void cpu_relax() {
#if defined(__x86_64__) || defined(__i386__)
    __builtin_ia32_pause();
#elif defined(__aarch64__)
    asm volatile("yield");
#endif
}

struct Core {
    Plan P;
    DevProblem d{};
    hipStream_t stream = nullptr;
    int device = 0;
    int n_cu = 256;
    rocblas_handle blas = nullptr;
    hipEvent_t ev[5] = {nullptr, nullptr, nullptr, nullptr, nullptr};
    hipEvent_t kev[13] = {};
    bool timing = false;
    struct { const void *kernel; size_t bytes; } lds_opt_in[8] = {};
    int n_lds_opt_in = 0;

    DevBuf<int32_t> cam_ncol, cam_col, cam_iorow, io_src, o_cam, o_pt;
    DevBuf<uint32_t> cam_eo_est, o_seg;
    DevBuf<double> io_fixed, px, cam_w, z_prw, z_prv, o_uv, o_w;
    bool pw = false;
    DevBuf<double> o_rhs;
    bool uv_pre = false;
    DevBuf<uint8_t> z_est, z_mine, o_lc, o_pidx;
    DevBuf<int64_t> o_row, batch_start, x2z, giant_start, cm_chunk_start;
    DevBuf<int32_t> cm_pt, cm_chunk_cam, tile_order;
    DevBuf<double> cm_uv, cm_w;
    int64_t n_cm_chunks = 0, n_cm_chunks_all = 0;
    int64_t nb = 0, nobs = 0;
    int grid_obs = 1, grid_z = 1, grid_zs = 1;
    size_t lds_build = 0, lds_back = 0, lds_cov = 0;
    bool deterministic = false;
    DevBuf<double> det_cam_part, det_io_part, det_rr, det_u;
    DevBuf<int32_t> det_cam_chunks;

    DevBuf<int32_t> tile_batch, tile_cam_start, tile_cams, tile_io_start, tile_iocols;
    DevBuf<uint8_t> tile_io_simple;
    DevBuf<uint8_t> tile_cam_io;
    DevBuf<int32_t> sg_chunk, sg_tile_chunk0, sg_gcam;
    int64_t sg_nchunks = 0;
    DevBuf<uint8_t> sg_lc;
    DevBuf<double> sg_uv, sg_w;
    int sig_rb = 4;
    int tile_ncx = 6;
    int64_t ntiles = 0;
    size_t lds_tile2 = 0, lds_tile3 = 0;
    enum class TileRoute { none, sig, tile3, tile2 } route = TileRoute::none;

    DevBuf<double> giant_W;
    int64_t ngiant = 0;
    bool use_heavy = false;
    HeavyDev hv{};
    DevBuf<int32_t> hv_obs_dst, hv_pt_io0, hv_io_dst, hv_io_pt, hv_pt_y, hv_grp_nb, hv_grp_row, hv_task, hv_ops;
    DevBuf<uint8_t> hv_obs_ld, hv_obs_ioloc, hv_io_ld;
    DevBuf<double> hv_Z;
    int giant_threads = 256;

    DevBuf<CamRec> cams, cams_f;
    bool cams_at_lin = false;
    const char *env_df_trace = nullptr;
    DevBuf<double> z, zt, dz, zlin, vtmp, vtmp2, xbuf;
    DevBuf<double> red;
    DevBuf<double> jn2c, dscale, rhs, Vinv, gp, jn2p;
    DevBuf<int> info;
    DevBuf<double> linv, ldiag;
    DataflowChol dfchol;
    DataflowChol dfchol_ip;
    bool use_perm = true;
    bool chol_in_place = false;
    int64_t ldS = 0;
    CholEnvelope env;
    DevBuf<unsigned long long> pivmm;
    double *S = nullptr, *g_red = nullptr, *g_c = nullptr, *diagU = nullptr, *red_scal = nullptr;
    int64_t red_count = 0;
    double f_lin = 0, trace_jtj = 0, lambda_lin = 0;
    int scale_lin = 0;
// ... 1601 lines not shown
```

dbat_amd/csrc/debug_host.hpp:

```cpp
#pragma once

extern "C" {
#define DBAT_PLAN_FIELDS(X)                                                                                           \
    X(x2z) X(io_src) X(io_fixed) X(z_est) X(z_prw) X(z_prv) X(z_mine) X(z0) X(prior_z) X(porder) X(pt_rank) X(o_cam)    \
    X(o_pt) X(o_uv) X(o_w) X(o_seg) X(o_row) X(batch_start) X(o_lc) X(o_pidx) X(tile_batch) X(tile_cam_start)           \
    X(tile_order) X(tile_cams) X(cm_pt) X(cm_uv) X(cm_w) X(cm_chunk_cam) X(cm_chunk_start) X(giant_start)               \
    X(tile_io_start) X(tile_iocols) X(tile_cam_io) X(tile_io_simple) X(sg_chunk) X(sg_tile_chunk0) X(sg_lc) X(sg_gcam)  \
    X(sg_uv) X(sg_w) X(cam_w) X(cam_ncol) X(cam_col) X(cam_iorow) X(cam_eo_est) X(px) X(cam_first) X(cam_adj)
int dbat_hip_debug_plan_digest(const dbat_hip_problem *prob, uint64_t *out, int32_t n_out, char *names, int32_t names_len) {
    API_TRY
    if (!prob || !out) { g_err = "null argument"; return DBAT_HIP_EINVAL; }
    Plan P;
    if (!build_plan(*prob, P, true)) { g_err = P.err; return DBAT_HIP_EINVAL; }
    auto fnv = [](const void *p, size_t n) {
        uint64_t h = 1469598103934665603ull;
        const unsigned char *b = (const unsigned char *)p;
        for (size_t i = 0; i < n; ++i) h = (h ^ b[i]) * 1099511628211ull;
        return h ^ (uint64_t)n;
    };
    std::vector<uint64_t> hs;
    std::string nm;
#define X(F) hs.push_back(fnv(P.F.data(), P.F.size() * sizeof(P.F[0]))); nm += #F ",";
    DBAT_PLAN_FIELDS(X)
#undef X
    hs.push_back(fnv(P.nd.order.data(), P.nd.order.size() * sizeof(int))); nm += "nd.order,";
    hs.push_back(fnv(P.nd.block_end.data(), P.nd.block_end.size() * sizeof(int))); nm += "nd.block_end,";
    hs.push_back(fnv(P.nd.cam_owner.data(), P.nd.cam_owner.size() * sizeof(int))); nm += "nd.cam_owner,";
    const int64_t sc[] = {P.n, P.m, P.NS, P.NZ, P.nIOu, P.pt_lo, P.pt_hi, P.CMAX, P.nb_tiled, P.n_cm_chunks_tiled, P.sg_kmax, P.sg_rows_max,
                          P.sg_ngroups, P.sg_npoints, P.sg_ok, P.sg_backsub_ok, P.BT, P.ncolmax, P.with_io, P.uniform_w, P.all_std8, P.max_k,
                          P.shared_eo, P.rank_ok, P.order_dims, P.mg_subtree, P.n_tiles_io_simple, P.n_prior[0], P.n_prior[1], P.n_prior[2]};
    hs.push_back(fnv(sc, sizeof(sc))); nm += "scalars";
    if ((int)hs.size() > n_out) { g_err = "digest buffer too small"; return DBAT_HIP_EINVAL; }
    for (size_t i = 0; i < hs.size(); ++i) out[i] = hs[i];
    for (int i = (int)hs.size(); i < n_out; ++i) out[i] = 0;
    if (names && names_len > 0) snprintf(names, (size_t)names_len, "%s", nm.c_str());
    return (int)hs.size();
    API_CATCH
}

int dbat_hip_debug_heavy_plan_selftest(const dbat_hip_problem *prob, double *out) {
    API_TRY
    if (!prob || !out) { g_err = "null argument"; return DBAT_HIP_EINVAL; }
    Plan P;
    if (!build_plan(*prob, P, true)) { g_err = P.err; return DBAT_HIP_EINVAL; }
    for (int i = 0; i < 8; ++i) out[i] = 0.0;
    if (!P.hv_ok) return DBAT_HIP_OK;
    const int64_t NS = P.NS;
    if (NS > 4000) { g_err = "selftest: reduced system too large for the dense host check"; return DBAT_HIP_EINVAL; }
    auto val = [](int64_t pt, int64_t row, int c) {
        uint64_t h = (uint64_t)pt * 0x9E3779B97F4A7C15ull ^ (uint64_t)(row + 1) * 0xC2B2AE3D27D4EB4Full ^ (uint64_t)(c + 1) * 0x165667B19E3779F9ull;
        h ^= h >> 29; h *= 0xBF58476D1CE4E5B9ull; h ^= h >> 32;
        return (double)(int64_t)(h % 2001) / 1000.0 - 1.0;
    };
    std::vector<double> Zs((size_t)P.hv_z_doubles, 0.0);
    std::vector<double> ref((size_t)(NS + 1) * (NS + 1), 0.0), got((size_t)(NS + 1) * (NS + 1), 0.0);
    const int64_t ho0 = P.hv_obs0, ho1 = (int64_t)P.o_cam.size();
    std::vector<int64_t> prow; std::vector<double> pval;
    int64_t o = ho0;
    while (o < ho1) {
        const int32_t pt = P.o_pt[o];
        const int32_t hp = pt - P.hv_pt0;
        prow.clear(); pval.clear();
        std::vector<int32_t> slot_row((size_t)(P.hv_pt_io0[hp + 1] - P.hv_pt_io0[hp]), -1);
        int64_t oe = o;
        for (; oe < ho1 && P.o_pt[oe] == pt; ++oe) {
            const int32_t c = P.o_cam[oe];
            const int32_t dst = P.hv_obs_dst[oe - ho0];
            const int ld = P.hv_obs_ld[oe - ho0];
            for (int a = 0; a < 6; ++a) {
                const int64_t row = P.cam_col[(size_t)c * MAXCOL + a];
                prow.push_back(row);
                for (int k = 0; k < 3; ++k) { const double v = val(pt, row, k); pval.push_back(v); Zs[(size_t)dst + (size_t)k * ld + a] = v; }
            }
            for (int q = 6; q < P.cam_ncol[c]; ++q) {
                const int sl = P.hv_obs_ioloc[(size_t)(oe - ho0) * Plan::HV_NIOC + (q - 6)];
                if (sl >= (int)slot_row.size()) { g_err = "selftest: IO slot out of range"; return DBAT_HIP_EINVAL; }
                const int32_t row = P.cam_col[(size_t)c * MAXCOL + q];
                if (slot_row[sl] >= 0 && slot_row[sl] != row) { g_err = "selftest: two IO columns in one slot"; return DBAT_HIP_EINVAL; }
                slot_row[sl] = row;
            }
        }
        for (size_t sl = 0; sl < slot_row.size(); ++sl) {
            if (slot_row[sl] < 0) { g_err = "selftest: IO slot without a column"; return DBAT_HIP_EINVAL; }
            const int gs = P.hv_pt_io0[hp] + (int)sl;
            if (P.hv_io_pt[gs] != hp) { g_err = "selftest: IO slot of another point"; return DBAT_HIP_EINVAL; }
            prow.push_back(slot_row[sl]);
            for (int k = 0; k < 3; ++k) { const double v = val(pt, slot_row[sl], k); pval.push_back(v); Zs[(size_t)P.hv_io_dst[gs] + (size_t)k * P.hv_io_ld[gs]] = v; }
        }
        prow.push_back(NS);
        for (int k = 0; k < 3; ++k) { const double v = val(pt, NS, k); pval.push_back(v); Zs[(size_t)P.hv_pt_y[2 * hp] + (size_t)k * P.hv_pt_y[2 * hp + 1]] = v; }
        for (size_t a = 0; a < prow.size(); ++a)
            for (size_t b = 0; b < prow.size(); ++b) {
                const int64_t ri = prow[a], rj = prow[b];
                if (ri < rj || (ri == NS && rj == NS)) continue;
                ref[(size_t)rj * (NS + 1) + ri] -= pval[3 * a] * pval[3 * b] + pval[3 * a + 1] * pval[3 * b + 1] + pval[3 * a + 2] * pval[3 * b + 2];
            }
        o = oe;
    }
    int64_t nks_all = 0;
    for (int t = 0; t < P.hv_ntasks; ++t) {
        const int gi = P.hv_task[4 * t], gj = P.hv_task[4 * t + 1], ks0 = P.hv_task[4 * t + 2], nks = P.hv_task[4 * t + 3];
        const int nbi = P.hv_grp_nb[gi], nbj = P.hv_grp_nb[gj];
        nks_all += nks;
        std::vector<double> acc((size_t)48 * 48, 0.0);
        for (int ks = 0; ks < nks; ++ks)
            for (int kk = 0; kk < 4; ++kk) {
                const int32_t *op = P.hv_ops.data() + ((size_t)(ks0 + ks) * 4 + kk) * 2;
                if ((op[0] < 0) != (op[1] < 0)) { g_err = "selftest: half an operand"; return DBAT_HIP_EINVAL; }
                if (op[0] < 0) continue;
                for (int i = 0; i < 16 * nbi; ++i)
                    for (int j = 0; j < 16 * nbj; ++j) acc[(size_t)i * 48 + j] += Zs[(size_t)op[0] + i] * Zs[(size_t)op[1] + j];
            }
        for (int i = 0; i < 16 * nbi; ++i)
            for (int j = 0; j < 16 * nbj; ++j) {
                if (gi == gj && i < j) continue;
                const int32_t ri = P.hv_grp_row[(size_t)gi * 48 + i], cj = P.hv_grp_row[(size_t)gj * 48 + j];
                if (ri < 0 || cj < 0 || cj == NS) continue;
                if (ri < cj) { g_err = "selftest: rows of the groups are not ascending"; return DBAT_HIP_EINVAL; }
                got[(size_t)cj * (NS + 1) + ri] -= acc[(size_t)i * 48 + j];
            }
    }
    double dmax = 0, vmax = 0; int64_t ncmp = 0;
    for (size_t i = 0; i < ref.size(); ++i) {
        dmax = std::max(dmax, std::fabs(ref[i] - got[i])); vmax = std::max(vmax, std::fabs(ref[i]));
        ncmp += ref[i] != 0.0;
    }
    out[0] = 1; out[1] = P.hv_npts; out[2] = P.hv_ngroups; out[3] = P.hv_ntasks; out[4] = (double)nks_all;
    out[5] = dmax; out[6] = vmax; out[7] = (double)ncmp;
    return DBAT_HIP_OK;
    API_CATCH
}

int dbat_hip_debug_batch_stats(const dbat_hip_problem *prob, int64_t *out) {
    API_TRY
    if (!prob || !out) { g_err = "null argument"; return DBAT_HIP_EINVAL; }
    Plan P;
    if (!build_plan(*prob, P, true)) { g_err = P.err; return DBAT_HIP_EINVAL; }
    for (int i = 0; i < 16; ++i) out[i] = 0;
    const int64_t nb = (int64_t)P.batch_start.size() - 1;
    for (int64_t b = 0; b < nb; ++b) {
        const int64_t o0 = P.batch_start[b], o1 = P.batch_start[b + 1];
        if (o1 <= o0) continue;
        int64_t *st = out + (b < P.nb_tiled ? 0 : 4);
        st[0] = std::max<int64_t>(st[0], (int64_t)P.o_pidx[o1 - 1] + 1);
        st[1] = std::max<int64_t>(st[1], o1 - o0);
    }
    out[2] = P.nb_pcap[0]; out[6] = P.nb_pcap[1];
    for (size_t t = 0; P.nb_tiled > 0 && t + 1 < P.tile_batch.size(); ++t)
        out[3] = std::max<int64_t>(out[3], P.tile_batch[t + 1] - P.tile_batch[t]);
    out[8] = P.BT; out[9] = Plan::PMAX; out[10] = P.tile_bmax; out[11] = P.nb_tiled; out[12] = nb - P.nb_tiled;
    return DBAT_HIP_OK;
    API_CATCH
}

int dbat_hip_debug_model_eval_host(int32_t model, int32_t nK, int32_t nP, const double *EO6, const double *IO,
                                   double px_size, const double *Q3, const double *uv, double *r2,
                                   double *A12, double *B6, double *C ) {
    if (model < 2 || model > 5 || nK < 0 || nK > MAXK || nP < 0 || nP > MAXP) { g_err = "bad model"; return DBAT_HIP_EINVAL; }
    CamRec c{};
    c.c[0] = EO6[0]; c.c[1] = EO6[1]; c.c[2] = EO6[2];
    cam_rotation(EO6 + 3, c.Mt, c.sk, c.ck);
    c.f = IO[0]; c.pp[0] = IO[1]; c.pp[1] = IO[2]; c.b[0] = IO[3]; c.b[1] = IO[4];
    for (int k = 0; k < nK; ++k) c.K[k] = IO[5 + k];
    for (int k = 0; k < nP; ++k) c.P[k] = IO[5 + nK + k];
    c.sz = px_size;
    double r[2], A[2][6], B[2][3], Cf[2][MAXIO];
    switch (model) {
        case 2: obs_eval<2, true, true>(c, nK, nP, Q3, uv[0], uv[1], r, A, B, Cf); break;
        case 3: obs_eval<3, true, true>(c, nK, nP, Q3, uv[0], uv[1], r, A, B, Cf); break;
        case 4: obs_eval<4, true, true>(c, nK, nP, Q3, uv[0], uv[1], r, A, B, Cf); break;
        default: obs_eval<5, true, true>(c, nK, nP, Q3, uv[0], uv[1], r, A, B, Cf); break;
    }
    r2[0] = r[0]; r2[1] = r[1];
    for (int k = 0; k < 6; ++k) { A12[2 * k] = A[0][k]; A12[2 * k + 1] = A[1][k]; }
    for (int k = 0; k < 3; ++k) { B6[2 * k] = B[0][k]; B6[2 * k + 1] = B[1][k]; }
    for (int k = 0; k < 5 + nK + nP; ++k) { C[2 * k] = Cf[0][k]; C[2 * k + 1] = Cf[1][k]; }
    return DBAT_HIP_OK;
}
}
```

dbat_amd/csrc/env.hpp:

```cpp
#pragma once
#include <cstdlib>
#include <cstring>
#include <string>

extern char **environ;

namespace dbat {

#ifdef DBAT_HIP_PROFILING
constexpr bool kProfilingBuild = true;
#else
constexpr bool kProfilingBuild = false;
#endif

struct EnvSwitch { const char *name; bool measurement; const char *what; const char *values = nullptr; };
static const EnvSwitch kEnvSwitches[] = {
    {"DBAT_HIP_SIG", false, "0: signature kernels off, 2: on wherever a chunk's rows fit (default: by group length)", "0|1|2"},
    {"DBAT_HIP_SIG_IOS_OFF", false, "self-calibration: IO rows by LDS atomics in every tile"},
    {"DBAT_HIP_CMAX", false, "cameras per tile (0: column-list kernel only)"},
    {"DBAT_HIP_BT", false, "observations per batch (128 | 256)", "128|256"},
    {"DBAT_HIP_TILE_BMIN", false, "fewest batches a tile may be capped at (default 2)"},
    {"DBAT_HIP_HEAVY", false, "0: heavy / giant points by the column-list kernels (pair terms by global atomics) instead of the matrix-core path", "0|1"},
    {"DBAT_HIP_HEAVY_KS", false, "heavy / giant points: k-steps per task of k_heavy_syrk at most (default: by the amount of work, 12 ... 96)"},
    {"DBAT_HIP_GIANT_THREADS", false, "threads of the giant-point kernels (64 | 128 | 256)", "64|128|256"},
    {"DBAT_HIP_MG_REPLICATED", false, "several ranks: envelope summed, replicated factorisation"},
    {"DBAT_HIP_ND_OFF", false, "no nested dissection"},
    {"DBAT_HIP_ND_LEAF", false, "leaf size of the dissection"},
    {"DBAT_HIP_ND_PAD_ALL", false, "every block of the dissection on a tile boundary"},
    {"DBAT_HIP_ND_JOIN_SMALL", false, "separators up to that many rows join their child's last tile"},
    {"DBAT_HIP_DF_SPLIT", false, "factorisation: helper tasks for sums longer than this many products (default 96)"},
    {"DBAT_HIP_DF_CHUNK", false, "factorisation: products per helper task (default 32)"},
    {"DBAT_HIP_DF_CHAIN", false, "factorisation: 0 = diagonal tiles as ordinary tasks (no chain role), 1 = chain role whatever the pattern", "0|1"},
    {"DBAT_HIP_DF_CHAIN_WG", false, "factorisation: workgroups of the chain role at most (default 32)"},
    {"DBAT_HIP_DF_L2", false, "factorisation: 1 = finished tiles of the compact layout are read through the L2", "0|1"},
    {"DBAT_HIP_COV_DENSE", false, "posterior covariance: the dense inverse of the reduced system (rocsolver_dpotri) instead of the selected inversion"},
    {"DBAT_HIP_SPRANK_OFF", false, "structural rank from the counting conditions only"},
    {"DBAT_HIP_PLAN_THREADS", false, "threads of the host plan (default: hardware concurrency, at most 32)"},
    {"DBAT_HIP_PLAN_GRAIN", false, "elements per thread below which a pass of the host plan is not split (tests: 1)"},
    {"DBAT_HIP_PLAN_STATS", false, "1: print layout statistics, 2: also the wall time of every section of the plan"},
    {"DBAT_HIP_PIVOT_STATS", false, "print the pivot extremes and the rcond estimate of every solve"},
    {"DBAT_HIP_ABLATE", true, "k_build_sig / tile kernels: switch phases off (results are wrong), phase clocks"},
    {"DBAT_HIP_DF_TRACE", true, "per-task clocks of the factorisation, written to this file"},
    {"DBAT_HIP_DF_TRACE_POTF2", true, "with DF_TRACE: clocks inside the chain role's factorisations as well"},
    {"DBAT_HIP_DF_ABLATE", true, "factorisation: operand tiles of the products not fetched (1: L(i,j), 2: both, 3: and no flag looks) -- timing only, wrong results", "0|1|2|3"},
    {"DBAT_HIP_DF_ORDER", true, "one of the candidate task orders instead of the simulated best"},
    {"DBAT_HIP_DF_GRID", true, "workgroups of the factorisation"},
    {"DBAT_HIP_GRID_OBS", true, "launch size of the observation-parallel kernels"},
};

inline const char *env_get(const char *name) {
    for (const EnvSwitch &e : kEnvSwitches)
        if (!strcmp(e.name, name)) return (e.measurement && !kProfilingBuild) ? nullptr : getenv(name);
    return nullptr;
}
inline int env_int(const char *name, int dflt) { const char *e = env_get(name); return e ? atoi(e) : dflt; }
inline bool env_on(const char *name) { return env_get(name) != nullptr; }

inline bool env_validate(std::string &err) {
    for (char **p = environ; p && *p; ++p) {
        if (strncmp(*p, "DBAT_HIP_", 9) != 0) continue;
        const char *eq = strchr(*p, '=');
        const std::string name(*p, eq ? (size_t)(eq - *p) : strlen(*p));
        const EnvSwitch *hit = nullptr;
        for (const EnvSwitch &e : kEnvSwitches) if (name == e.name) hit = &e;
        if (!hit) { err = "unknown environment variable " + name + " (the switches of libdbat_hip.so: csrc/env.hpp, DESIGN.md 9)"; return false; }
        if (hit->measurement && !kProfilingBuild) {
            err = name + " is a measurement switch (" + hit->what + "): this library was built without -DDBAT_HIP_PROFILING (make -C dbat_amd/csrc prof)";
            return false;
        }
        if (hit->values && eq) {
            const std::string val(eq + 1), list = std::string("|") + hit->values + "|";
            if (val.empty() || val.find('|') != std::string::npos || list.find("|" + val + "|") == std::string::npos) {
                err = name + "=" + val + ": not one of " + hit->values + " (" + hit->what + ")";
                return false;
            }
        }
    }
    return true;
}

}
```

dbat_amd/csrc/nd.hpp:

```cpp
#pragma once
#include <algorithm>
#include <cstdint>
#include <functional>
#include <vector>

namespace dbat {

struct NdTree {
    int nparts = 1;
    std::vector<int> order;
    std::vector<int> block_end;
    std::vector<int> block_owner;
    std::vector<uint8_t> block_sep;
    std::vector<int> cam_owner;
    int n_top_cams = 0;
};

inline void nd_build(int nc, const uint64_t *adj, int adj_words, const double *xyz, const double *weight,
                     int nparts, int leaf, bool nd_off, NdTree &T) {
    T = NdTree();
    T.nparts = std::max(1, nparts);
    T.order.reserve(nc);
    T.cam_owner.assign(nc, 0);
    auto adjacent = [&](int a, int b) { return (adj[(size_t)a * adj_words + (b >> 6)] >> (b & 63)) & 1ull; };
    auto emit = [&](std::vector<int> &cams, int owner, bool sep = false) {
        std::sort(cams.begin(), cams.end());
        for (int c : cams) { T.order.push_back(c); T.cam_owner[c] = owner; if (owner < 0) ++T.n_top_cams; }
        if (!cams.empty()) { T.block_end.push_back((int)T.order.size()); T.block_owner.push_back(owner); T.block_sep.push_back(sep ? 1 : 0); }
    };
    std::function<void(std::vector<int> &, int, int)> nd = [&](std::vector<int> &cams, int part0, int np) {
        if (cams.empty()) return;
        if (np == 1 && (int)cams.size() <= leaf) { emit(cams, part0); return; }
        double lo[3] = {1e300, 1e300, 1e300}, hi[3] = {-1e300, -1e300, -1e300};
        for (int c : cams) for (int d = 0; d < 3; ++d) { lo[d] = std::min(lo[d], xyz[3 * c + d]); hi[d] = std::max(hi[d], xyz[3 * c + d]); }
        int ax = 0;
        for (int d = 1; d < 3; ++d) if (hi[d] - lo[d] > hi[ax] - lo[ax]) ax = d;
        std::vector<int> s(cams);
        std::stable_sort(s.begin(), s.end(), [&](int a, int b) { return xyz[3 * a + ax] < xyz[3 * b + ax]; });
        size_t half = s.size() / 2;
        const int npa = np / 2, npb = np - npa;
        std::vector<int> A, B, Sep, A2;
        auto cut = [&](size_t h) {
            A.assign(s.begin(), s.begin() + h); B.assign(s.begin() + h, s.end()); Sep.clear(); A2.clear();
            for (int a : A) {
                bool touch = false;
                for (int b : B) if (adjacent(a, b)) { touch = true; break; }
                (touch ? Sep : A2).push_back(a);
            }
        };
        if (np > 1) {
            auto wsum = [&](const std::vector<int> &v) { double t = 0; for (int c : v) t += weight ? weight[c] : 1.0; return t; };
            size_t lo = 1, hi = s.size() - 1;
            half = std::min(std::max<size_t>(s.size() * npa / np, lo), hi);
            for (int it = 0; it < 16 && lo < hi; ++it) {
                cut(half);
                const double wa = wsum(A2) / npa, wb = wsum(B) / npb;
                if (wa < wb) lo = half + 1; else hi = half;
                const size_t next = (lo + hi) / 2;
                if (next == half) break;
                half = next;
            }
            half = std::min(std::max<size_t>(half, 1), s.size() - 1);
        }
        cut(half);
        if (Sep.size() * 2 >= cams.size() || A2.empty()) {
            emit(cams, np > 1 ? -1 : part0);
            return;
        }
        nd(A2, part0, np > 1 ? npa : 1);
        nd(B, np > 1 ? part0 + npa : part0, np > 1 ? npb : 1);
        emit(Sep, np > 1 ? -1 : part0, true);
    };
    std::vector<int> all(nc);
    for (int c = 0; c < nc; ++c) all[c] = c;
    if (nd_off) emit(all, T.nparts > 1 ? -1 : 0);
    else nd(all, 0, T.nparts);
}

}
```

dbat_amd/csrc/plan.hpp:

```cpp
#pragma once
#include "env.hpp"
#include "par.hpp"
#include <atomic>
#include <chrono>
#include <algorithm>
#include <cmath>
#include <cstdint>
#include <cstdlib>
#include <cstring>
#include <numeric>
#include <string>
#include <unordered_map>
#include <vector>

#include "../../include/dbat_hip.h"
#include "model.hpp"
#include "nd.hpp"

namespace dbat {

struct Plan {
    int nc = 0, np = 0, nIOrows = 0, nK = 0, nP = 0, model = 0;
    int64_t no = 0;
    int rank = 0, nranks = 1;
    int64_t n = 0, nIO = 0, nEO = 0, nOP = 0;
    int64_t NS = 0, NZ = 0;
    int nIOu = 0;
    std::vector<int64_t> x2z;
    std::vector<int64_t> lead_io;
    uint64_t key[2] = {0, 0};
    std::vector<int32_t> io_src;
    std::vector<double> io_fixed;
    std::vector<uint8_t> z_est;
    std::vector<double> z_prw, z_prv;
    std::vector<uint8_t> z_mine;
    std::vector<double> z0;
    std::vector<int64_t> prior_z;
    int64_t n_prior[3] = {0, 0, 0};
    int64_t m = 0;
    int64_t pt_lo = 0, pt_hi = 0;
    std::vector<int32_t> porder;
    std::vector<int32_t> pt_rank;
    uvec<int32_t> o_cam, o_pt;
    uvec<double> o_uv;
    uvec<double> o_w;
    uvec<uint32_t> o_seg;
    uvec<int64_t> o_row;
    std::vector<int64_t> batch_start;
    static constexpr int PMAX = 128;
    int64_t nb_pcap[2] = {0, 0};
    int tile_bmax = 0;
    uvec<uint8_t> o_lc;
    uvec<uint8_t> o_pidx;
    std::vector<int32_t> tile_batch;
    std::vector<int32_t> tile_cam_start;
    std::vector<int32_t> tile_order;
    std::vector<int32_t> tile_cams;
    int CMAX = 0;
    int64_t nb_tiled = 0;
    static constexpr int CM_CHUNK = 2048;
    uvec<int32_t> cm_pt;
    uvec<double> cm_uv;
    uvec<double> cm_w;
    std::vector<int32_t> cm_chunk_cam;
    std::vector<int64_t> cm_chunk_start;
    int64_t n_cm_chunks_tiled = 0;
    std::vector<int64_t> giant_start;
    static constexpr int IOT = 16;
    std::vector<int32_t> tile_io_start;
    std::vector<int32_t> tile_iocols;
    std::vector<uint8_t> tile_cam_io;
    std::vector<uint8_t> tile_io_simple;
    int32_t n_tiles_io_simple = 0;
    static constexpr int SG_KMAX = 13;
#ifndef DBAT_SIG_IO_WAVES
#define DBAT_SIG_IO_WAVES 4
#endif
    static constexpr int SIG_IO_CMAX = DBAT_SIG_IO_WAVES == 8 ? 16 : 18;
    static constexpr int SG_CHUNK = 64;
    std::vector<int32_t> sg_chunk;
    std::vector<int32_t> sg_tile_chunk0;
    std::vector<uint8_t> sg_lc;
    std::vector<int32_t> sg_gcam;
    uvec<double> sg_uv;
    uvec<double> sg_w;
    int sg_kmax = 0;
    int sg_rows_max = 0;
    int64_t sg_ngroups = 0, sg_npoints = 0;
    bool sg_ok = false;
    bool sg_backsub_ok = false;
    int BT = 256;
    int ncolmax = 6;
    bool with_io = false;
    bool uniform_w = true;
    std::vector<double> cam_w;
    std::vector<int32_t> cam_ncol, cam_col, cam_iorow;
    std::vector<uint32_t> cam_eo_est;
    bool all_std8 = false;
    std::vector<double> px;
    std::vector<int32_t> cam_first;
    std::vector<uint64_t> cam_adj;
    int cam_adj_words = 0;
    NdTree nd;
    bool mg_subtree = false;
    int max_k = 0;
    bool shared_eo = false;
    bool rank_ok = true;
    bool tang_zero = false;
    bool hv_ok = false;
    int64_t hv_obs0 = 0;
    int32_t hv_pt0 = 0, hv_npts = 0;
    int32_t hv_ngroups = 0, hv_ntasks = 0, hv_ks_per_task = 0;
    int64_t hv_z_doubles = 0;
    int64_t hv_mfma = 0;
    int64_t hv_alg_flops = 0;
    int hv_max_io_slots = 0;
    int hv_max_batch_slots = 0;
    std::vector<int32_t> hv_grp_nb;
    std::vector<int32_t> hv_grp_row;
    std::vector<int32_t> hv_obs_dst;
    std::vector<uint8_t> hv_obs_ld;
    std::vector<uint8_t> hv_obs_ioloc;
    std::vector<int32_t> hv_pt_io0;
    std::vector<int32_t> hv_io_dst;
    std::vector<uint8_t> hv_io_ld;
    std::vector<int32_t> hv_io_pt;
    std::vector<int32_t> hv_pt_y;
    std::vector<int32_t> hv_task;
    std::vector<int32_t> hv_ops;
    static constexpr int HV_NIOC = 9;
    static constexpr int HV_MAXSLOTS = 48;
    int order_dims = 3;
    std::string err;
};

inline bool fail(Plan &P, const std::string &msg) { P.err = msg; return false; }

inline void serialize_block(int rows, int cols, const int32_t *block, const uint8_t *est,
                            std::vector<int32_t> &dist, std::vector<int64_t> &lead_entries,
                            bool &simple) {
    dist.assign((size_t)rows * cols, -1);
    std::vector<uint8_t> leading((size_t)rows * cols, 0);
    simple = true;
    for (int i = 0; i < rows; ++i) {
        std::unordered_map<int32_t, int> seen;
        for (int j = 0; j < cols; ++j) {
            const size_t e = (size_t)j * rows + i;
            if (!est[e] || block[e] == 0) continue;
            if (seen.emplace(block[e], j).second) leading[e] = 1;
            else simple = false;
        }
    }
    lead_entries.clear();
    for (size_t e = 0; e < leading.size(); ++e)
        if (leading[e]) { dist[e] = (int32_t)lead_entries.size(); lead_entries.push_back((int64_t)e); }
    if (!simple) {
        for (int i = 0; i < rows; ++i) {
            std::unordered_map<int32_t, int32_t> lead_of;
            for (int j = 0; j < cols; ++j) {
                const size_t e = (size_t)j * rows + i;
                if (leading[e]) lead_of[block[e]] = dist[e];
            }
            for (int j = 0; j < cols; ++j) {
                const size_t e = (size_t)j * rows + i;
                if (!est[e] || block[e] == 0 || leading[e]) continue;
                dist[e] = lead_of[block[e]];
            }
        }
    }
}

inline void build_heavy_plan(Plan &P) {
    P.hv_ok = false; P.hv_ntasks = 0; P.hv_ngroups = 0; P.hv_z_doubles = 0; P.hv_mfma = 0;
    if (!P.CMAX || P.BT != 256 || P.shared_eo || P.ncolmax > 6 + Plan::HV_NIOC) return;
    if (env_int("DBAT_HIP_HEAVY", 1) == 0) return;
    const int64_t nb = (int64_t)P.batch_start.size() - 1;
    if (P.nb_tiled > nb) return;
    const int64_t ho0 = P.batch_start[P.nb_tiled], ho1 = (int64_t)P.o_cam.size();
    if (ho1 <= ho0) return;
    const int nc = P.nc;
    const int32_t hp0 = P.o_pt[ho0], hp1 = P.o_pt[ho1 - 1] + 1;
    const int32_t nhp = hp1 - hp0;
    std::vector<int64_t> pobs((size_t)nhp + 1, ho1);
    for (int64_t o = ho1 - 1; o >= ho0; --o) pobs[P.o_pt[o] - hp0] = o;
    for (int32_t i = nhp - 1; i >= 0; --i) if (pobs[i] > pobs[i + 1]) pobs[i] = pobs[i + 1];
    std::vector<int32_t> cam_idx((size_t)nc, -1), hcams;
    for (int64_t o = ho0; o < ho1; ++o) cam_idx[P.o_cam[o]] = 0;
    for (int c = 0; c < nc; ++c) if (cam_idx[c] == 0) { cam_idx[c] = (int32_t)hcams.size(); hcams.push_back(c); }
    std::vector<int32_t> io_idx((size_t)std::max(1, P.nIOu), -1), hio;
    for (int32_t c : hcams)
        for (int q = 6; q < P.cam_ncol[c]; ++q) io_idx[P.cam_col[(size_t)c * MAXCOL + q] - 6 * nc] = 0;
    for (int k = 0; k < P.nIOu; ++k) if (io_idx[k] == 0) { io_idx[k] = (int32_t)hio.size(); hio.push_back(k); }
    const int ngc = ((int)hcams.size() + 7) / 8;
    const int nior = (int)hio.size() + 1;
    const int ngi = (nior + 47) / 48;
    const int ng = ngc + ngi;
    P.hv_ngroups = ng;
    P.hv_grp_nb.assign(ng, 0); P.hv_grp_row.assign((size_t)ng * 48, -1);
    for (size_t i = 0; i < hcams.size(); ++i)
        for (int a = 0; a < 6; ++a) P.hv_grp_row[(i / 8) * 48 + 6 * (i % 8) + a] = 6 * hcams[i] + a;
    for (int i = 0; i < nior; ++i)
        P.hv_grp_row[(size_t)(ngc + i / 48) * 48 + i % 48] = i < (int)hio.size() ? 6 * nc + hio[i] : (int32_t)P.NS;
    for (int g = 0; g < ng; ++g) {
        int rows = 0;
        for (int r = 0; r < 48; ++r) if (P.hv_grp_row[(size_t)g * 48 + r] >= 0) rows = r + 1;
        P.hv_grp_nb[g] = (rows + 15) / 16;
    }
    const int yg = ngc + (nior - 1) / 48, yrow = (nior - 1) % 48;
    std::vector<int32_t> cnt((size_t)ng, 0);
    std::vector<int64_t> pg0((size_t)nhp + 1, 0);
    std::vector<int32_t> pg_g, pg_slot;
    const int64_t nho = ho1 - ho0;
    P.hv_obs_dst.assign((size_t)nho, 0); P.hv_obs_ld.assign((size_t)nho, 16);
    P.hv_obs_ioloc.assign((size_t)nho * Plan::HV_NIOC, 255);
    P.hv_pt_io0.assign((size_t)nhp + 1, 0); P.hv_io_dst.clear(); P.hv_io_ld.clear(); P.hv_io_pt.clear();
    P.hv_pt_y.assign((size_t)2 * nhp, 0);
    P.hv_max_io_slots = 0;
    std::vector<int32_t> pio;
    std::vector<int32_t> grp_slot((size_t)ng, -1);
    std::vector<int32_t> touched;
    std::vector<int32_t> io_slot_grp;
    for (int32_t i = 0; i < nhp; ++i) {
        pio.clear(); touched.clear();
        for (int64_t o = pobs[i]; o < pobs[i + 1]; ++o) {
            const int32_t c = P.o_cam[o];
            const int g = cam_idx[c] / 8;
            if (grp_slot[g] < 0) { grp_slot[g] = cnt[g]++; touched.push_back(g); }
            for (int q = 6; q < P.cam_ncol[c]; ++q) pio.push_back(io_idx[P.cam_col[(size_t)c * MAXCOL + q] - 6 * nc]);
        }
        std::sort(pio.begin(), pio.end());
        pio.erase(std::unique(pio.begin(), pio.end()), pio.end());
        if ((int)pio.size() > Plan::HV_MAXSLOTS) return;
        P.hv_max_io_slots = std::max(P.hv_max_io_slots, (int)pio.size());
        for (int32_t q : pio) { const int g = ngc + q / 48; if (grp_slot[g] < 0) { grp_slot[g] = cnt[g]++; touched.push_back(g); } }
        if (pobs[i + 1] > pobs[i] && grp_slot[yg] < 0) { grp_slot[yg] = cnt[yg]++; touched.push_back(yg); }
        std::sort(touched.begin(), touched.end());
        for (int32_t g : touched) { pg_g.push_back(g); pg_slot.push_back(grp_slot[g]); }
        pg0[i + 1] = (int64_t)pg_g.size();
        for (int64_t o = pobs[i]; o < pobs[i + 1]; ++o) {
            const int32_t c = P.o_cam[o];
            const int g = cam_idx[c] / 8, ld = 16 * P.hv_grp_nb[g];
            P.hv_obs_dst[o - ho0] = grp_slot[g] * 3 * ld + 6 * (cam_idx[c] % 8);
            P.hv_obs_ld[o - ho0] = (uint8_t)ld;
            for (int q = 6; q < P.cam_ncol[c]; ++q) {
                const int32_t io = io_idx[P.cam_col[(size_t)c * MAXCOL + q] - 6 * nc];
                P.hv_obs_ioloc[(size_t)(o - ho0) * Plan::HV_NIOC + (q - 6)] = (uint8_t)(std::lower_bound(pio.begin(), pio.end(), io) - pio.begin());
            }
        }
        for (int32_t q : pio) {
            const int g = ngc + q / 48, ld = 16 * P.hv_grp_nb[g];
            P.hv_io_dst.push_back(grp_slot[g] * 3 * ld + q % 48);
            P.hv_io_ld.push_back((uint8_t)ld); P.hv_io_pt.push_back(i); io_slot_grp.push_back(g);
        }
        P.hv_pt_io0[i + 1] = (int32_t)P.hv_io_dst.size();
        if (pobs[i + 1] > pobs[i]) { const int ld = 16 * P.hv_grp_nb[yg]; P.hv_pt_y[2 * i] = grp_slot[yg] * 3 * ld + yrow; P.hv_pt_y[2 * i + 1] = ld; }
        for (int32_t g : touched) grp_slot[g] = -1;
// ... 445 lines not shown
                for (int dd = 0; dd < 2 * k && want > 0; ++dd) {
                    const int j = (int)((p + dd) % k);
                    const int64_t row = 2 * by_pt[pstart[p] + j] + (dd >= k ? 1 : 0);
                    __atomic_fetch_or(&taken[row >> 6], 1ull << (row & 63), __ATOMIC_RELAXED);
                    --want;
                }
                if (want > 0) { short_pts.fetch_add(1); return; }
            }
        });
        bool cheap_ok = short_pts.load() == 0;
        auto claim = [&](int c, int64_t &row) -> bool {
            while (row < 2 * cam_obs0[c + 1] && ((taken[row >> 6] >> (row & 63)) & 1)) ++row;
            if (row >= 2 * cam_obs0[c + 1]) return false;
            taken[row >> 6] |= 1ull << (row & 63);
            return true;
        };
        if (cheap_ok) {
            std::vector<uint8_t> io_done(std::max(1, P.nIOu), 0);
            int64_t io_left = 0;
            for (int k = 0; k < P.nIOu; ++k) { io_done[k] = !wanted(6 * (int64_t)nc + k); io_left += !io_done[k]; }
            for (int c = 0; c < nc && io_left > 0; ++c) {
                int64_t row = 2 * cam_obs0[c];
                for (int r = 0; r < R && io_left > 0; ++r) {
                    const int32_t k = distIO[(size_t)c * R + r];
                    if (k < 0 || io_done[k]) continue;
                    if (!claim(c, row)) break;
                    io_done[k] = 1; --io_left;
                }
            }
            cheap_ok = io_left == 0;
        }
        for (int c = 0; c < nc && cheap_ok; ++c) {
            int64_t row = 2 * cam_obs0[c];
            for (int d = 0; d < 6 && cheap_ok; ++d)
                if (wanted(6 * (int64_t)c + d)) cheap_ok = claim(c, row);
        }
        sprank_settled = cheap_ok;
    }
    lapt("structural rank: cheap assignment in parallel");
    if (plan_clock) fprintf(stderr, "[plan clock] cheap assignment settled the structural rank: %s\n", sprank_settled ? "yes" : "no");
    if (P.rank_ok && !sprank_settled && !env_on("DBAT_HIP_SPRANK_OFF") && !P.shared_eo) {
        const int64_t ncol_all = P.NZ;
        std::vector<int64_t> cam_obs0(nc + 1, 0);
        for (int c = 0; c < nc; ++c) cam_obs0[c + 1] = cam_obs0[c] + n_cam[c];
        std::vector<std::vector<int32_t>> io_cams(P.nIOu);
        std::vector<std::vector<int64_t>> io_cum(P.nIOu);
        for (int c = 0; c < nc; ++c)
            for (int r = 0; r < R; ++r) {
                const int32_t s = distIO[(size_t)c * R + r];
                if (s >= 0 && n_cam[c] > 0) io_cams[s].push_back(c);
            }
        for (int k = 0; k < P.nIOu; ++k) {
            io_cum[k].assign(io_cams[k].size() + 1, 0);
            for (size_t i = 0; i < io_cams[k].size(); ++i) io_cum[k][i + 1] = io_cum[k][i] + 2 * (int64_t)n_cam[io_cams[k][i]];
        }
        const int64_t eo_end = 6 * (int64_t)nc, io_end = P.NS;
        auto nrows = [&](int64_t col) -> int64_t {
            if (col < eo_end) return 2 * (int64_t)n_cam[col / 6];
            if (col < io_end) return io_cum[col - eo_end].back();
            return 2 * (int64_t)k_pt[(col - io_end) / 3];
        };
        auto row_at = [&](int64_t col, int64_t i) -> int64_t {
            if (col < eo_end) return 2 * cam_obs0[col / 6] + i;
            if (col < io_end) {
                const auto &cum = io_cum[col - eo_end];
                const size_t q = std::upper_bound(cum.begin(), cum.end(), i) - cum.begin() - 1;
                return 2 * cam_obs0[io_cams[col - eo_end][q]] + (i - cum[q]);
            }
            const int64_t p = (col - io_end) / 3;
            return 2 * by_pt[pstart[p] + (i >> 1)] + (i & 1);
        };
        std::vector<int32_t> row_owner((size_t)2 * P.no, -1);
        std::vector<int64_t> cheap(ncol_all, 0), iter(ncol_all, 0), take(ncol_all, -1);
        std::vector<int32_t> stamp(ncol_all, -1);
        std::vector<int64_t> stack;
        int32_t gen = 0;
        auto match_column = [&](int64_t k) -> bool {
            stack.assign(1, k); iter[k] = 0; stamp[k] = ++gen;
            while (!stack.empty()) {
                const int64_t j = stack.back(), nr = nrows(j);
                bool found = false;
                while (cheap[j] < nr) {
                    const int64_t r = row_at(j, cheap[j]++);
                    if (row_owner[r] < 0) { take[j] = r; found = true; break; }
                }
                if (found) {
                    for (int64_t c : stack) row_owner[take[c]] = (int32_t)c;
                    return true;
                }
                bool deeper = false;
                while (iter[j] < nr) {
                    const int64_t r = row_at(j, iter[j]++), j2 = row_owner[r];
                    if (stamp[j2] != gen) {
                        stamp[j2] = gen; take[j] = r; iter[j2] = 0;
                        stack.push_back(j2); deeper = true;
                        break;
                    }
                }
                if (!deeper) stack.pop_back();
            }
            return false;
        };
        auto wanted = [&](int64_t col) -> bool { return P.z_est[col] && !(P.z_prw[col] > 0); };
        for (int64_t col = eo_end; col < io_end && P.rank_ok; ++col) if (wanted(col) && !match_column(col)) P.rank_ok = false;
        for (int64_t col = 0; col < eo_end && P.rank_ok; ++col) if (wanted(col) && !match_column(col)) P.rank_ok = false;
        for (int64_t col = io_end; col < ncol_all && P.rank_ok; ++col) if (wanted(col) && !match_column(col)) P.rank_ok = false;
    }

    lapt("structural rank: exact matching (only when the cheap assignment fails)");
    P.cam_first.resize(nc);
    for (int c = 0; c < nc; ++c) P.cam_first[c] = c;
    P.cam_adj_words = (nc + 63) / 64;
    P.cam_adj.assign((size_t)nc * P.cam_adj_words, 0);
    {
        const size_t aw = (size_t)nc * P.cam_adj_words;
        const int nr = (int)std::min<int64_t>(par.ranges(np, 1 << 14), std::max<int64_t>(1, (int64_t)(256u << 20) / (int64_t)std::max<size_t>(aw * 8, 1)));
        std::vector<std::vector<uint64_t>> adj_t(nr);
        std::vector<std::vector<int32_t>> first_t(nr);
        const Par par_adj{nr};
        par_adj.run(np, [&](int64_t plo, int64_t phi, int tid) {
            std::vector<uint64_t> &adj = adj_t[tid];
            std::vector<int32_t> &first = first_t[tid];
            adj.assign(aw, 0); first.resize(nc);
            for (int c = 0; c < nc; ++c) first[c] = c;
            for (int64_t p = plo; p < phi; ++p) {
                const int k = k_pt[p];
                if (!k) continue;
                const int32_t *cp = cbp.data() + pstart[p];
                const int32_t c0 = cp[0];
                for (int j = 1; j < k; ++j) if (c0 < first[cp[j]]) first[cp[j]] = c0;
                for (int a = 0; a < k; ++a) {
                    uint64_t *row = adj.data() + (size_t)cp[a] * P.cam_adj_words;
                    for (int b = 0; b < k; ++b) row[cp[b] >> 6] |= 1ull << (cp[b] & 63);
                }
            }
        }, 1);
        for (int t = 0; t < nr; ++t) {
            if (adj_t[t].empty()) continue;
            for (size_t i = 0; i < aw; ++i) P.cam_adj[i] |= adj_t[t][i];
            for (int c = 0; c < nc; ++c) P.cam_first[c] = std::min(P.cam_first[c], first_t[t][c]);
        }
    }
    lapt("camera co-visibility graph");
    {
        const bool nd_off = env_on("DBAT_HIP_ND_OFF");
        const bool permuted_ok = !P.shared_eo;
        P.mg_subtree = P.nranks > 1 && permuted_ok && !nd_off && !env_on("DBAT_HIP_MG_REPLICATED");
        std::vector<double> xyz((size_t)3 * nc), wcam(nc);
        for (int c = 0; c < nc; ++c) {
            for (int k = 0; k < 3; ++k) { const double v = pb.EO_val[(size_t)6 * c + k]; xyz[(size_t)3 * c + k] = std::isfinite(v) ? v : 0.0; }
            wcam[c] = (double)n_cam[c];
        }
        const int leaf = std::max(8, env_int("DBAT_HIP_ND_LEAF", 32));
        nd_build(nc, P.cam_adj.data(), P.cam_adj_words, xyz.data(), wcam.data(), P.mg_subtree ? P.nranks : 1, leaf, nd_off, P.nd);
    }
    lapt("nested dissection");
    P.CMAX = env_int("DBAT_HIP_CMAX", P.with_io ? Plan::SIG_IO_CMAX : 21);
    if (P.shared_eo) P.CMAX = 0;
    if (P.CMAX < 0 || P.CMAX > (P.with_io ? 18 : 21)) P.CMAX = P.with_io ? 18 : 21;
    if (P.ncolmax > 15) P.CMAX = 0;
    {
        P.BT = env_int("DBAT_HIP_BT", 256);
        if (P.BT != 128 && P.BT != 256) P.BT = 256;
        if ((size_t)P.BT * P.ncolmax * 3 * 8 + (size_t)P.BT * 18 * 8 > 150 * 1024) P.BT = 128;
        if (P.BT != 256) P.CMAX = 0;
    }
    std::vector<uint8_t> heavy(np, 0), giant(np, 0);
    par.run(np, [&](int64_t plo, int64_t phi, int) {
    for (int64_t p = plo; p < phi; ++p) giant[p] = k_pt[p] > P.BT;
    for (int64_t p = plo; p < phi && P.CMAX; ++p) {
        if (k_pt[p] > P.CMAX) { heavy[p] = 1; continue; }
        if (P.with_io) {
            int32_t seen[Plan::IOT + 1]; int ns = 0;
            for (int j = 0; j < k_pt[p] && ns <= Plan::IOT; ++j) {
                const int32_t c = cbp[pstart[p] + j];
                for (int q = 6; q < P.cam_ncol[c] && ns <= Plan::IOT; ++q) {
                    const int32_t io = P.cam_col[(size_t)c * MAXCOL + q];
                    bool f = false;
                    for (int t = 0; t < ns; ++t) if (seen[t] == io) { f = true; break; }
                    if (!f) seen[ns++] = io;
                }
            }
            if (ns > Plan::IOT) heavy[p] = 1;
        }
    }
    });
    {
        int64_t n_heavy = 0, n_tiled = 0;
        for (int p = 0; p < np; ++p) { if (giant[p]) continue; if (heavy[p]) n_heavy += k_pt[p]; else n_tiled += k_pt[p]; }
        const bool hv_can = P.CMAX && P.BT == 256 && !P.shared_eo && P.ncolmax <= 6 + Plan::HV_NIOC && env_int("DBAT_HIP_HEAVY", 1) != 0;
        if (hv_can && n_heavy > 0 && n_tiled <= 2048)
            for (int p = 0; p < np; ++p) if (k_pt[p] > 0 && !giant[p]) heavy[p] = 1;
    }
    lapt("tile-fit classification of the points");
    std::vector<uint64_t> key(np);
    {
        double mean[3] = {0, 0, 0}, cov[3][3] = {{0, 0, 0}, {0, 0, 0}, {0, 0, 0}};
        int64_t nfin = 0;
        for (int p = 0; p < np; ++p) {
            const double *q = pb.OP_val + (size_t)3 * p;
            if (std::isfinite(q[0]) && std::isfinite(q[1]) && std::isfinite(q[2])) { ++nfin; for (int d = 0; d < 3; ++d) mean[d] += q[d]; }
        }
        for (int d = 0; d < 3; ++d) mean[d] /= (double)std::max<int64_t>(nfin, 1);
        for (int p = 0; p < np; ++p) {
            const double *q = pb.OP_val + (size_t)3 * p;
            if (!(std::isfinite(q[0]) && std::isfinite(q[1]) && std::isfinite(q[2]))) continue;
            for (int i = 0; i < 3; ++i) for (int j = 0; j < 3; ++j) cov[i][j] += (q[i] - mean[i]) * (q[j] - mean[j]);
        }
        double ax[3][3] = {{1, 0, 0}, {0, 1, 0}, {0, 0, 1}};
        for (int sweep = 0; sweep < 30; ++sweep) {
            const double off = std::fabs(cov[0][1]) + std::fabs(cov[0][2]) + std::fabs(cov[1][2]);
            if (!(off > 1e-14 * (std::fabs(cov[0][0]) + std::fabs(cov[1][1]) + std::fabs(cov[2][2])))) break;
            for (int i = 0; i < 2; ++i)
                for (int j = i + 1; j < 3; ++j) {
                    if (cov[i][j] == 0.0) continue;
                    const double th = 0.5 * std::atan2(2 * cov[i][j], cov[j][j] - cov[i][i]);
                    const double cs = std::cos(th), sn = std::sin(th);
                    for (int k = 0; k < 3; ++k) {
                        const double a = cov[k][i], b = cov[k][j];
                        cov[k][i] = cs * a - sn * b; cov[k][j] = sn * a + cs * b;
                    }
                    for (int k = 0; k < 3; ++k) {
                        const double a = cov[i][k], b = cov[j][k];
                        cov[i][k] = cs * a - sn * b; cov[j][k] = sn * a + cs * b;
                    }
                    for (int k = 0; k < 3; ++k) {
                        const double a = ax[k][i], b = ax[k][j];
                        ax[k][i] = cs * a - sn * b; ax[k][j] = sn * a + cs * b;
                    }
                }
        }
        auto coord = [&](int p, int a) {
            const double *q = pb.OP_val + (size_t)3 * p;
            return (q[0] - mean[0]) * ax[0][a] + (q[1] - mean[1]) * ax[1][a] + (q[2] - mean[2]) * ax[2][a];
        };
        double lo[3] = {1e300, 1e300, 1e300}, hi[3] = {-1e300, -1e300, -1e300};
        for (int p = 0; p < np; ++p)
            for (int d = 0; d < 3; ++d) {
                const double v = coord(p, d);
                if (std::isfinite(v)) { lo[d] = std::min(lo[d], v); hi[d] = std::max(hi[d], v); }
            }
        int axis[3] = {0, 1, 2};
        std::sort(axis, axis + 3, [&](int a, int b) { return hi[a] - lo[a] > hi[b] - lo[b]; });
        double ext = hi[axis[0]] - lo[axis[0]];
        if (!(ext > 0)) ext = 1;
        const int dims = (hi[axis[2]] - lo[axis[2]]) < 0.2 * ext ? 2 : 3;
        P.order_dims = dims;
        auto spread = [](uint64_t v) {
            v &= 0x1FFFFF;
            v = (v | v << 32) & 0x1F00000000FFFFull;
            v = (v | v << 16) & 0x1F0000FF0000FFull;
            v = (v | v << 8) & 0x100F00F00F00F00Full;
            v = (v | v << 4) & 0x10C30C30C30C30C3ull;
            v = (v | v << 2) & 0x1249249249249249ull;
            return v;
        };
        par.run(np, [&](int64_t plo, int64_t phi, int) {
            for (int64_t p = plo; p < phi; ++p) {
                uint64_t k = 0;
                for (int d = 0; d < dims; ++d) {
                    double v = (coord((int)p, axis[d]) - lo[axis[d]]) / ext;
                    if (!(v >= 0)) v = 0;
                    if (v > 1) v = 1;
                    k |= spread((uint64_t)(v * 2097151.0)) << d;
                }
                key[p] = !k_pt[p] ? ~0ull
                         : giant[p] ? ((k >> 2) | (3ull << 62))
                         : heavy[p] ? ((k >> 2) | (1ull << 63)) : (k >> 1);
            }
        });
    }
    P.porder.resize(np);
    std::iota(P.porder.begin(), P.porder.end(), 0);
    {
        int64_t nobs_pts = 0;
        for (int p = 0; p < np; ++p) nobs_pts += k_pt[p] > 0;
        int cell_bits = 0;
        while (((int64_t)512 << cell_bits) < nobs_pts && cell_bits < 60) ++cell_bits;
        const int eff_bits = (cell_bits * 3 + P.order_dims - 1) / P.order_dims;
        const int low_bits = std::max(0, 62 - eff_bits);
        struct Rec { uint64_t cell, sig, key; int32_t p; };
        std::vector<Rec> recs(np);
        par.run(np, [&](int64_t plo, int64_t phi, int) {
            for (int64_t p = plo; p < phi; ++p) {
                uint64_t sg = 0;
                const bool in_cell = low_bits > 0 && key[p] < (1ull << 62);
                if (in_cell) {
                    uint64_t lead = 0, h = 1469598103934665603ull;
                    for (int j = 0; j < k_pt[p]; ++j) {
                        const uint64_t c = (uint64_t)cbp[pstart[p] + j];
                        if (j < 3) lead |= (c & 0xFFFF) << (48 - 16 * j);
                        h = (h ^ c) * 1099511628211ull;
                    }
                    sg = lead | (h & 0xFFFF);
                }
                recs[p] = Rec{in_cell ? key[p] >> low_bits : key[p], sg, key[p], (int32_t)p};
            }
        });
        par.sort(recs, [](const Rec &a, const Rec &b) {
            if (a.cell != b.cell) return a.cell < b.cell;
            if (a.sig != b.sig) return a.sig < b.sig;
            if (a.key != b.key) return a.key < b.key;
            return a.p < b.p;
        });
        par.run(np, [&](int64_t lo_, int64_t hi_, int) { for (int64_t i = lo_; i < hi_; ++i) P.porder[i] = recs[i].p; });
    }
    if (P.mg_subtree) {
// ... 426 lines not shown
```

Baseline: 628.6.

## Select nested-dissection separators by modelled Cholesky cost and cut sums at merge columns

Adds alternative separator modes for nested dissection: minimum vertex cover and slid cuts. They are scored with a host-side model of the Cholesky schedule, and the cheapest ordering is kept. It also optionally rebuilds the dataflow job list with partial sums split at elimination-tree merge columns, adopted when the simulated schedule is shorter. The aim is to cut the sparse Cholesky critical path and fill per LM iteration, at the cost of extra planning work and more partial-sum buffers.

After: 645.3, median of 6. +2.7%, better.

```diff
diff --git a/dbat_amd/_hip.py b/dbat_amd/_hip.py
--- a/dbat_amd/_hip.py
+++ b/dbat_amd/_hip.py
@@ -201,6 +201,7 @@
     'dbat_hip_debug_plan_digest': (C.c_int, [C.POINTER(Problem), C.POINTER(C.c_uint64), C.c_int32, C.c_char_p, C.c_int32]),
     'dbat_hip_debug_heavy_plan_selftest': (C.c_int, [C.POINTER(Problem), _dp]),
     'dbat_hip_debug_batch_stats': (C.c_int, [C.POINTER(Problem), C.POINTER(C.c_int64)]),
+    'dbat_hip_debug_nd_stats': (C.c_int, [C.POINTER(Problem), C.c_int32, _dp]),
     'dbat_hip_debug_model_eval_host': (C.c_int, [C.c_int32, C.c_int32, C.c_int32, _dp, _dp, C.c_double,
                                                  _dp, _dp, _dp, _dp, _dp, _dp]),
     'dbat_hip_debug_ray_angles_ms': (C.c_int, [_H, _dp, C.POINTER(C.c_int64)]),
@@ -1000,6 +1001,17 @@
                 max_diff=float(out[5]), max_abs=float(out[6]), entries=int(out[7]))
 
 
+def nd_stats(s, mode, shard_rank=0, shard_count=1):
+    lib = load()
+    p, keep = problem_from_struct(s, 0, shard_rank, shard_count)
+    out = np.zeros(24)
+    check(lib.dbat_hip_debug_nd_stats(C.byref(p), int(mode), dptr(out)))
+    part = lambda v: dict(cameras=int(v[0]), blocks=int(v[1]), tile_columns=int(v[2]), tiles=int(v[3]), chain=int(v[4]),
+                          products=int(v[5]), model_us=float(v[6]), mode=int(v[7]), valid=int(v[8]) == 0, run=int(v[9]),
+                          model='estimate' if v[10] else 'list schedule')
+    return part(out[:12]), part(out[12:])
+
+
 def batch_stats(s, shard_rank=0, shard_count=1):
     lib = load()
     p, keep = problem_from_struct(s, 0, shard_rank, shard_count)
diff --git a/dbat_amd/csrc/chol_df.hpp b/dbat_amd/csrc/chol_df.hpp
--- a/dbat_amd/csrc/chol_df.hpp
+++ b/dbat_amd/csrc/chol_df.hpp
@@ -1099,7 +1099,7 @@
         return true;
     }
     struct JobList { std::vector<DfJob> jobs; std::vector<int> dptr, dep, own, sumjob, presum, bits, par; };
-    void build_jobs(int phase, const std::vector<uint64_t> &rowbits, const std::vector<int> &col_owner, int rank, JobList &L) {
+    void build_jobs(int phase, const std::vector<uint64_t> &rowbits, const std::vector<int> &col_owner, int rank, JobList &L, int merge_depth = 0) {
         auto has = [&](int i, int k) { return (rowbits[(size_t)i * W + (k >> 6)] >> (k & 63)) & 1ull; };
         const int split_min = std::max(env_int("DBAT_HIP_DF_SPLIT", 96), 2);
         const int chunk = std::max(env_int("DBAT_HIP_DF_CHUNK", 32), 1);
@@ -1115,15 +1115,47 @@
         const bool chain = use_chain && merge;
         auto inphase = [&](int c) { return c < nT && (phase == 0 || (phase == 1 ? col_owner[c] == rank : col_owner[c] < 0)); };
         std::vector<int> js;
+        const int merge_min = 4;
+        int merge_k = 0;
+        int run0 = 0;
+        std::vector<int> run_of(nT, 0), merge_cut;
         for (int k = 0; k < nT; ++k) {
+            if (chain && merge_depth > 0) {
+                if (!(k > 0 && (L.bits[k - 1] & 2))) { run0 = k; merge_cut.clear(); }
+                run_of[k] = run0;
+                int c = run0 - 1;
+                while (c >= 0 && L.par[c] != k) --c;
+                if (c >= 0) { merge_cut.assign({run_of[c], c + 1, run0}); merge_k = k; }
+                else if (k - merge_k >= merge_depth) merge_cut.clear();
+            }
             auto emit = [&](int i, int mode, int par, int jhi_owner) {
-                n_products += (long long)js.size();
-                const int nj = (int)js.size();
-                const int nch = nj > split_min ? (nj + chunk - 1) / chunk : 1;
                 auto push_products = [&](int q0, int q1) {
                     for (int q = q0; q < q1; ++q) { L.dep.push_back(L.own[(size_t)k * nT + js[q]]); L.dep.push_back(i != k ? L.own[(size_t)i * nT + js[q]] : -1); }
                     L.dptr.push_back((int)L.dep.size());
                 };
+                n_products += (long long)js.size();
+                const int nj = (int)js.size();
+                const int nch = nj > split_min ? (nj + chunk - 1) / chunk : 1;
+                if (nch == 1 && !merge_cut.empty()) {
+                    int qc[4], npc = 0, q0 = 0;
+                    for (int c : merge_cut) {
+                        const int q = (int)(std::lower_bound(js.begin(), js.end(), c) - js.begin());
+                        if (q > q0) { qc[npc++] = q; q0 = q; }
+                    }
+                    if (npc > 0 && nj - q0 >= merge_min) {
+                        q0 = 0;
+                        for (int c = 0; c < npc; ++c) {
+                            L.jobs.push_back(DfJob{i, k, js[q0], qc[c] < nj ? js[qc[c]] : jhi_owner, nparts + c, -1, 0, -1});
+                            push_products(q0, qc[c]);
+                            q0 = qc[c];
+                        }
+                        const int me = (int)L.jobs.size();
+                        L.jobs.push_back(DfJob{i, k, q0 < nj ? js[q0] : jhi_owner, jhi_owner, nparts, npc, mode, i == k ? par : -1});
+                        push_products(q0, nj);
+                        nparts += npc;
+                        return me;
+                    }
+                }
                 for (int c = 0; c + 1 < nch; ++c) {
                     L.jobs.push_back(DfJob{i, k, js[chunk * c], js[chunk * (c + 1)], nparts + c, -1, 0, -1});
                     push_products(chunk * c, chunk * (c + 1));
@@ -1258,6 +1290,7 @@
         std::vector<double> key(nt), tcs(ncand);
         const int forced = env_int("DBAT_HIP_DF_ORDER", -1);
         for (int c = 0; c < ncand; ++c) {
+            if (quiet && forced < 0 && c != 0 && c != 3) { tcs[c] = 1e300; continue; }
             if (c + 1 < ncand) for (int t = 0; t < nt; ++t) key[t] = est[t] - betas[c] * blev[t];
             else for (int t = 0; t < nt; ++t) key[t] = est[t] - c_prod * nprod_of(t);
             std::vector<int> ord = kahn(key);
@@ -1267,7 +1300,7 @@
         double cp = 0.0;
         for (int t = 0; t < nt; ++t) cp = std::max(cp, fin[t]);
         sim_critical_us.push_back(cp); sim_schedule_us.push_back(tbest);
-        if (env_on("DBAT_HIP_PLAN_STATS")) {
+        if (stats_on()) {
             fprintf(stderr, "[chol %s] %d tasks, critical path %.0f us; simulated with %d workgroups, key = earliest start - beta x bottom level:",
                     what, nt, cp, workers);
             for (int c = 0; c + 1 < ncand; ++c) fprintf(stderr, " beta %g: %.0f us,", betas[c], tcs[c]);
@@ -1277,8 +1310,10 @@
         for (int t = 0; t < nt; ++t) sorted[t] = jobs[best_ord[t]];
         jobs.swap(sorted);
     }
-    bool finish_setup(const std::vector<uint64_t> &rowbits, const std::vector<int64_t> &toff,
-                      const std::vector<int> &col_owner = std::vector<int>(), int rank = 0) {
+    struct Sched { std::vector<int> colsA, colsB, bitsA, bitsB, par, pos, bkl, bptr, bidx; std::vector<uint64_t> rowbits_top; };
+    bool quiet = false;
+    bool stats_on() const { return !quiet && env_on("DBAT_HIP_PLAN_STATS"); }
+    void schedule_host(const std::vector<uint64_t> &rowbits, const std::vector<int> &col_owner, int rank, Sched &H) {
         auto has = [&](int i, int k) { return (rowbits[(size_t)i * W + (k >> 6)] >> (k & 63)) & 1ull; };
         if (const char *g = env_get("DBAT_HIP_DF_GRID")) grid = std::min(std::max(atoi(g), 1), 4096);
         nparts = 0; n_products = 0;
@@ -1306,7 +1341,7 @@
             }
             const double t_products = (double)nprod * 2.6 / std::min(grid, 256), t_chain = longest * 17.0;
             use_chain = t_products < 0.6 * t_chain;
-            if (env_on("DBAT_HIP_PLAN_STATS"))
+            if (stats_on())
                 fprintf(stderr, "[chol] %lld tile products (%.0f us over the workgroups), longest chain %d links (%.0f us): chain role %s\n",
                         nprod, t_products, longest, t_chain, use_chain ? "on" : "off");
         }
@@ -1322,14 +1357,27 @@
             for (int k : cols) runs += !(bits[k] & 1);
             return std::max(1, std::min(runs, env_int("DBAT_HIP_DF_CHAIN_WG", 32)));
         };
-        std::vector<int> colsA, colsB;
+        std::vector<int> &colsA = H.colsA, &colsB = H.colsB;
         sim_critical_us.clear(); sim_schedule_us.clear();
         JobList L;
-        std::vector<int> bkl;
-        std::vector<uint64_t> rowbits_top;
+        std::vector<int> &bkl = H.bkl;
+        bkl.clear(); h_tasksB.clear(); ntasksB = 0; nchain = nchainB = 0; chain_wg = chain_wgB = 0;
         if (!two_phase) {
             build_jobs(0, rowbits, col_owner, rank, L);
             order_jobs(L, "all");
+            const int force_merge = env_int("DBAT_HIP_DF_MERGE", -1);
+            if (use_chain && force_merge != 0) {
+                const int np0 = nparts;
+                const long long prod0 = n_products;
+                JobList M;
+                nparts = 0; n_products = 0;
+                build_jobs(0, rowbits, col_owner, rank, M, 2);
+                order_jobs(M, "all, sums cut at the merge columns");
+                const bool better = nparts <= 4096 && (force_merge == 1 || sim_schedule_us[1] < 0.99 * sim_schedule_us[0]);
+                if (better) std::swap(L, M); else { nparts = np0; n_products = prod0; }
+                sim_critical_us.erase(sim_critical_us.begin() + (better ? 0 : 1)); sim_schedule_us.erase(sim_schedule_us.begin() + (better ? 0 : 1));
+                if (stats_on()) fprintf(stderr, "[chol] sums cut at the merge columns: %s (%d partial sums)\n", better ? "yes" : "no", nparts);
+            }
             split_chain(L, h_tasks, colsA); ntasks = (int)h_tasks.size();
             for (int j = nT - 1; j >= 0; --j) bkl.push_back(j);
         } else {
@@ -1340,28 +1388,26 @@
             build_jobs(2, rowbits, col_owner, rank, B);
             order_jobs(B, "top");
             split_chain(B, h_tasksB, colsB); ntasksB = (int)h_tasksB.size();
-            if (!up(d_tasksB, h_tasksB)) return false;
             if (use_chain) {
                 for (int k = 0; k < nT; ++k) if (B.par[k] >= 0) L.par[k] = B.par[k];
                 nchainB = (int)colsB.size(); chain_wgB = chain_width(colsB, B.bits);
-                if (!up(d_chain_colsB, colsB) || !up(d_chain_bitsB, B.bits)) return false;
+                H.bitsB = B.bits;
             }
             for (int j = nT - 1; j >= 0; --j) if (col_owner[j] < 0) bkl.push_back(j);
             for (int j = nT - 1; j >= 0; --j) if (col_owner[j] == rank) bkl.push_back(j);
-            rowbits_top = rowbits;
+            H.rowbits_top = rowbits;
             for (int i = 0; i <= nT; ++i)
                 for (int k = 0; k < nT; ++k)
-                    if (col_owner[k] >= 0) rowbits_top[(size_t)i * W + (k >> 6)] &= ~(1ull << (k & 63));
-            if (!up(d_rowbits_top, rowbits_top)) return false;
+                    if (col_owner[k] >= 0) H.rowbits_top[(size_t)i * W + (k >> 6)] &= ~(1ull << (k & 63));
         }
         nbk = (int)bkl.size();
         if (use_chain) {
             nchain = (int)colsA.size(); chain_wg = chain_width(colsA, L.bits);
-            std::vector<int> pos(nT, 0);
-            for (size_t q = 0; q < colsA.size(); ++q) pos[colsA[q]] = (int)q;
-            for (size_t q = 0; q < colsB.size(); ++q) pos[colsB[q]] = (int)q;
-            if (!up(d_chain_cols, colsA) || !up(d_chain_bits, L.bits) || !up(d_chain_par, L.par) || !up(d_chain_pos, pos)) return false;
-            if (env_on("DBAT_HIP_PLAN_STATS")) {
+            H.pos.assign(nT, 0);
+            for (size_t q = 0; q < colsA.size(); ++q) H.pos[colsA[q]] = (int)q;
+            for (size_t q = 0; q < colsB.size(); ++q) H.pos[colsB[q]] = (int)q;
+            H.bitsA = L.bits; H.par = L.par;
+            if (stats_on()) {
                 int runs = 0, longest = 0, cur = 0;
                 for (int k = 0; k < nT; ++k) { if (L.bits[k] & 1) ++cur; else { cur = 1; } longest = std::max(longest, cur); }
                 for (int k : colsA) runs += !(L.bits[k] & 1);
@@ -1369,14 +1415,24 @@
                         two_phase ? " (domain)" : "");
             }
         }
-        if (env_on("DBAT_HIP_DF_TRACE") && !two_phase && hipMalloc(&d_trace, (size_t)(ntasks + 3 * nT) * 16 * sizeof(long long)) != hipSuccess) d_trace = nullptr;
-        std::vector<int> bptr(nT + 1, 0), bidx;
+        H.bptr.assign(nT + 1, 0); H.bidx.clear();
         for (int j = 0; j < nT; ++j) {
             for (int i = nT - 1; i > j; --i)
-                if (has(i, j)) bidx.push_back(i);
-            bptr[j + 1] = (int)bidx.size();
-        }
-        if (!up(d_tasks, h_tasks) || !up(d_bk_ptr, bptr) || !up(d_bk_idx, bidx) || !up(d_rowbits, rowbits) || !up(d_toff, toff) || !up(d_bk_list, bkl))
+                if (has(i, j)) H.bidx.push_back(i);
+            H.bptr[j + 1] = (int)H.bidx.size();
+        }
+    }
+    bool finish_setup(const std::vector<uint64_t> &rowbits, const std::vector<int64_t> &toff,
+                      const std::vector<int> &col_owner = std::vector<int>(), int rank = 0) {
+        Sched H;
+        schedule_host(rowbits, col_owner, rank, H);
+        if (two_phase) {
+            if (!up(d_tasksB, h_tasksB) || !up(d_rowbits_top, H.rowbits_top)) return false;
+            if (use_chain && (!up(d_chain_colsB, H.colsB) || !up(d_chain_bitsB, H.bitsB))) return false;
+        }
+        if (use_chain && (!up(d_chain_cols, H.colsA) || !up(d_chain_bits, H.bitsA) || !up(d_chain_par, H.par) || !up(d_chain_pos, H.pos))) return false;
+        if (env_on("DBAT_HIP_DF_TRACE") && !two_phase && hipMalloc(&d_trace, (size_t)(ntasks + 3 * nT) * 16 * sizeof(long long)) != hipSuccess) d_trace = nullptr;
+        if (!up(d_tasks, h_tasks) || !up(d_bk_ptr, H.bptr) || !up(d_bk_idx, H.bidx) || !up(d_rowbits, rowbits) || !up(d_toff, toff) || !up(d_bk_list, H.bkl))
             return false;
         if (hipMalloc(&d_flags, ((size_t)(nT + 1) * nT + (size_t)nparts + 4 * (size_t)nT) * sizeof(int)) != hipSuccess) return false;
         if (nparts > 0 && hipMalloc(&d_parts, (size_t)nparts * 4096 * sizeof(double)) != hipSuccess) return false;
@@ -1403,8 +1459,68 @@
         }
         return finish_setup(rb, toff);
     }
+    struct Symbolic {
+        std::vector<int> iperm, col_owner;
+        std::vector<uint64_t> rb;
+        std::vector<int64_t> toff;
+        std::vector<DfTask> tile_ij;
+    };
+    struct PatternStats { int etree_depth = 0, longest_run = 0; long long products = 0; };
+    PatternStats pattern_stats(const std::vector<uint64_t> &rb) const {
+        PatternStats st;
+        std::vector<int> depth(nT, 1);
+        int cur = 0;
+        for (int k = 0; k < nT; ++k) {
+            int par = -1;
+            for (int i = k + 1; i < nT; ++i) {
+                if (!((rb[(size_t)i * W + (k >> 6)] >> (k & 63)) & 1ull)) continue;
+                if (par < 0) par = i;
+                for (int w = 0; w <= (k >> 6); ++w) {
+                    uint64_t m = rb[(size_t)i * W + w] & rb[(size_t)k * W + w];
+                    if (w == (k >> 6)) m &= (1ull << (k & 63)) - 1;
+                    st.products += __builtin_popcountll(m);
+                }
+            }
+            for (int w = 0; w <= (k >> 6); ++w) {
+                uint64_t m = rb[(size_t)k * W + w];
+                if (w == (k >> 6)) m &= (1ull << (k & 63)) - 1;
+                st.products += __builtin_popcountll(m);
+            }
+            st.etree_depth = std::max(st.etree_depth, depth[k]);
+            if (par >= 0) depth[par] = std::max(depth[par], depth[k] + 1);
+            cur = cur > 0 ? cur : 1;
+            st.longest_run = std::max(st.longest_run, cur);
+            cur = par == k + 1 ? cur + 1 : 0;
+        }
+        return st;
+    }
     bool setup_permuted(int nc, int nio, const uint64_t *adj, int adj_words, const NdTree &nd, int rank) {
         release();
+        Symbolic Y;
+        symbolic_permuted(nc, nio, adj, adj_words, nd, Y);
+        const std::vector<int> &block_end = nd.block_end;
+        if (!up(d_tile_ij, Y.tile_ij) || !up(d_iperm, Y.iperm)) return false;
+        if (hipMalloc(&d_tiles, (size_t)ntiles * 4096 * sizeof(double)) != hipSuccess) return false;
+        (void)hipMemset(d_tiles, 0, (size_t)ntiles * 4096 * sizeof(double));
+        if (hipMalloc(&d_qperm, (size_t)nT * CHOL_NB * sizeof(double)) != hipSuccess) return false;
+        if (env_on("DBAT_HIP_PLAN_STATS"))
+            fprintf(stderr, "[chol] order %d (%d with block padding, %zu blocks), %d tile rows, %d tiles (%.1f MB), dense lower triangle would be %d tiles\n",
+                    n_nat, n, block_end.size(), nT, ntiles, ntiles * 32768.0 / 1e6, nT * (nT + 1) / 2 + nT);
+        if (env_on("DBAT_HIP_PLAN_STATS")) {
+            fprintf(stderr, "[chol] cameras per block, last (root separator) first:");
+            for (size_t b = block_end.size(); b-- > 0 && block_end.size() - b <= 24;)
+                fprintf(stderr, " %d", block_end[b] - (b ? block_end[b - 1] : 0));
+            fprintf(stderr, "\n");
+        }
+        if (env_on("DBAT_HIP_PLAN_STATS") && !Y.col_owner.empty()) {
+            int ntop = 0, nmine = 0;
+            for (int k = 0; k < nT; ++k) { ntop += Y.col_owner[k] < 0; nmine += Y.col_owner[k] == rank; }
+            fprintf(stderr, "[chol] rank %d of %d: %d tile columns in its domain, %d top columns, %lld top tiles (%.1f MB summed over the ranks per factorisation)\n",
+                    rank, nd.nparts, nmine, ntop, (long long)n_top_tiles, n_top_tiles * 32768.0 / 1e6);
+        }
+        return finish_setup(Y.rb, Y.toff, Y.col_owner, rank);
+    }
+    void symbolic_permuted(int nc, int nio, const uint64_t *adj, int adj_words, const NdTree &nd, Symbolic &Y) {
         permuted = true;
         n_nat = 6 * nc + nio;
         const std::vector<int> &order = nd.order, &block_end = nd.block_end;
@@ -1430,13 +1546,15 @@
         n = (io0 + nio + CHOL_NB - 1) / CHOL_NB * CHOL_NB;
         nT = n / CHOL_NB; W = (nT + 64) / 64;
         perm.assign(n_nat, 0);
-        std::vector<int> iperm((size_t)n, -1);
+        std::vector<int> &iperm = Y.iperm;
+        iperm.assign((size_t)n, -1);
         for (int c = 0; c < nc; ++c)
             for (int a = 0; a < 6; ++a) perm[6 * c + a] = rowpos[c] + a;
         for (int u = 0; u < nio; ++u) perm[6 * nc + u] = io0 + u;
         for (int z = 0; z < n_nat; ++z) iperm[perm[z]] = z;
         auto pos6 = [&](int c) { return rowpos[c]; };
-        std::vector<uint64_t> rb((size_t)(nT + 1) * W, 0);
+        std::vector<uint64_t> &rb = Y.rb;
+        rb.assign((size_t)(nT + 1) * W, 0);
         auto setbit = [&](int i, int k) { rb[(size_t)i * W + (k >> 6)] |= 1ull << (k & 63); };
         for (int a = 0; a < nc; ++a) {
             const int ta0 = pos6(a) / CHOL_NB, ta1 = (pos6(a) + 5) / CHOL_NB;
@@ -1466,7 +1584,8 @@
                         if (rows[b] < nT) setbit(rows[a], rows[b]);
             }
         }
-        std::vector<int> col_owner;
+        std::vector<int> &col_owner = Y.col_owner;
+        col_owner.clear();
         if (nd.nparts > 1) {
             col_owner.assign(nT, -1);
             size_t b = 0;
@@ -1476,8 +1595,9 @@
                 for (int t = rowpos[order[q]] / CHOL_NB; t <= (rowpos[order[q]] + 5) / CHOL_NB; ++t) col_owner[t] = ow;
             }
         }
-        std::vector<int64_t> toff((size_t)(nT + 1) * nT, -1);
-        std::vector<DfTask> tile_ij;
+        std::vector<int64_t> &toff = Y.toff;
+        std::vector<DfTask> &tile_ij = Y.tile_ij;
+        toff.assign((size_t)(nT + 1) * nT, -1); tile_ij.clear();
         for (int pass = 0; pass < 2; ++pass) {
             if (pass == 1) top_tile0 = (int64_t)tile_ij.size();
             for (int k = 0; k < nT; ++k) {
@@ -1491,26 +1611,6 @@
         }
         ntiles = (int)tile_ij.size();
         n_top_tiles = ntiles - top_tile0;
-        if (!up(d_tile_ij, tile_ij) || !up(d_iperm, iperm)) return false;
-        if (hipMalloc(&d_tiles, (size_t)ntiles * 4096 * sizeof(double)) != hipSuccess) return false;
-        (void)hipMemset(d_tiles, 0, (size_t)ntiles * 4096 * sizeof(double));
-        if (hipMalloc(&d_qperm, (size_t)nT * CHOL_NB * sizeof(double)) != hipSuccess) return false;
-        if (env_on("DBAT_HIP_PLAN_STATS"))
-            fprintf(stderr, "[chol] order %d (%d with block padding, %zu blocks), %d tile rows, %d tiles (%.1f MB), dense lower triangle would be %d tiles\n",
-                    n_nat, n, block_end.size(), nT, ntiles, ntiles * 32768.0 / 1e6, nT * (nT + 1) / 2 + nT);
-        if (env_on("DBAT_HIP_PLAN_STATS")) {
-            fprintf(stderr, "[chol] cameras per block, last (root separator) first:");
-            for (size_t b = block_end.size(); b-- > 0 && block_end.size() - b <= 24;)
-                fprintf(stderr, " %d", block_end[b] - (b ? block_end[b - 1] : 0));
-            fprintf(stderr, "\n");
-        }
-        if (env_on("DBAT_HIP_PLAN_STATS") && !col_owner.empty()) {
-            int ntop = 0, nmine = 0;
-            for (int k = 0; k < nT; ++k) { ntop += col_owner[k] < 0; nmine += col_owner[k] == rank; }
-            fprintf(stderr, "[chol] rank %d of %d: %d tile columns in its domain, %d top columns, %lld top tiles (%.1f MB summed over the ranks per factorisation)\n",
-                    rank, nd.nparts, nmine, ntop, (long long)n_top_tiles, n_top_tiles * 32768.0 / 1e6);
-        }
-        return finish_setup(rb, toff, col_owner, rank);
     }
     bool selinv_supported() const { return permuted && !two_phase; }
     bool selected_inverse(hipStream_t stream, const double *linv_work) {
@@ -1626,4 +1726,23 @@
     }
 };
 
-}
+inline void df_score_order(int nc, int nio, const uint64_t *adj, int adj_words, const NdTree &T, NdScore &sc) {
+    DataflowChol D;
+    D.quiet = true;
+    DataflowChol::Symbolic Y;
+    D.symbolic_permuted(nc, nio, adj, adj_words, T, Y);
+    const DataflowChol::PatternStats st = D.pattern_stats(Y.rb);
+    sc.cams = nc; sc.blocks = (int)T.block_end.size(); sc.tile_cols = D.nT; sc.tiles = D.ntiles;
+    sc.chain = st.etree_depth; sc.run = st.longest_run; sc.products = st.products;
+    if (st.products > 1000000) {
+        sc.model = 1;
+        sc.model_us = std::max(st.etree_depth * 17.0, (double)st.products * 2.6 / std::min(D.grid, 256));
+    } else {
+        DataflowChol::Sched H;
+        D.schedule_host(Y.rb, std::vector<int>(), 0, H);
+        sc.model = 0;
+        sc.model_us = D.sim_schedule_us.empty() ? 0.0 : D.sim_schedule_us[0];
+    }
+}
+
+}
diff --git a/dbat_amd/csrc/dbat_core.hip b/dbat_amd/csrc/dbat_core.hip
--- a/dbat_amd/csrc/dbat_core.hip
+++ b/dbat_amd/csrc/dbat_core.hip
@@ -35,6 +35,8 @@
 namespace dbat {
 
 static thread_local std::string g_err;
+
+static const bool g_nd_score_registered = (nd_score_hook() = df_score_order, true);
 
 struct DeviceError { std::string msg; };
 struct UsageError { std::string msg; };
diff --git a/dbat_amd/csrc/debug_host.hpp b/dbat_amd/csrc/debug_host.hpp
--- a/dbat_amd/csrc/debug_host.hpp
+++ b/dbat_amd/csrc/debug_host.hpp
@@ -153,6 +153,30 @@
     API_CATCH
 }
 
+int dbat_hip_debug_nd_stats(const dbat_hip_problem *prob, int32_t mode, double *out) {
+    API_TRY
+    if (!prob || !out || mode < 0 || mode > 2) { g_err = "null argument or mode not 0, 1, 2"; return DBAT_HIP_EINVAL; }
+    Plan P;
+    if (!build_plan(*prob, P, false)) { g_err = P.err; return DBAT_HIP_EINVAL; }
+    const bool nd_off = env_on("DBAT_HIP_ND_OFF");
+    const int nparts = P.mg_subtree ? P.nranks : 1;
+    auto put = [&](const NdTree &T, NdScore sc, int m, double *o) {
+        if (sc.mode != m) df_score_order(P.nc, P.nIOu, P.cam_adj.data(), P.cam_adj_words, T, sc);
+        const double v[12] = {(double)sc.cams, (double)sc.blocks, (double)sc.tile_cols, (double)sc.tiles, (double)sc.chain, (double)sc.products,
+                              sc.model_us, (double)m, (double)nd_check(P.nc, P.cam_adj.data(), P.cam_adj_words, T), (double)sc.run, (double)sc.model, 0.0};
+        std::copy(v, v + 12, o);
+    };
+    NdTree T;
+    nd_build(P.nc, P.cam_adj.data(), P.cam_adj_words, P.nd_xyz.data(), P.nd_weight.data(), nparts, P.nd_leaf, nd_off, mode, T);
+    put(T, NdScore(), mode, out);
+    NdScore sc[3];
+    const int chosen = nd_select(P.nc, P.nIOu, P.cam_adj.data(), P.cam_adj_words, P.nd_xyz.data(), P.nd_weight.data(), nparts, P.nd_leaf, nd_off,
+                                 -1, true, T, sc);
+    put(T, sc[chosen], chosen, out + 12);
+    return DBAT_HIP_OK;
+    API_CATCH
+}
+
 int dbat_hip_debug_model_eval_host(int32_t model, int32_t nK, int32_t nP, const double *EO6, const double *IO,
                                    double px_size, const double *Q3, const double *uv, double *r2,
                                    double *A12, double *B6, double *C ) {
diff --git a/dbat_amd/csrc/env.hpp b/dbat_amd/csrc/env.hpp
--- a/dbat_amd/csrc/env.hpp
+++ b/dbat_amd/csrc/env.hpp
@@ -26,11 +26,13 @@
     {"DBAT_HIP_MG_REPLICATED", false, "several ranks: envelope summed, replicated factorisation"},
     {"DBAT_HIP_ND_OFF", false, "no nested dissection"},
     {"DBAT_HIP_ND_LEAF", false, "leaf size of the dissection"},
+    {"DBAT_HIP_ND_SEP", false, "separators inside a domain: 0 = lower boundary at the median, 1 = minimum vertex cover at the median, 2 = minimum cover with slid cuts (default: the one the model of the factorisation prefers)", "0|1|2"},
     {"DBAT_HIP_ND_PAD_ALL", false, "every block of the dissection on a tile boundary"},
     {"DBAT_HIP_ND_JOIN_SMALL", false, "separators up to that many rows join their child's last tile"},
     {"DBAT_HIP_DF_SPLIT", false, "factorisation: helper tasks for sums longer than this many products (default 96)"},
     {"DBAT_HIP_DF_CHUNK", false, "factorisation: products per helper task (default 32)"},
     {"DBAT_HIP_DF_CHAIN", false, "factorisation: 0 = diagonal tiles as ordinary tasks (no chain role), 1 = chain role whatever the pattern", "0|1"},
+    {"DBAT_HIP_DF_MERGE", false, "factorisation: sums of the columns where two parts of the dissection meet cut into early and late pieces: 0 = never, 1 = wherever the chain role is on (default: where the simulated schedule is shorter)", "0|1"},
     {"DBAT_HIP_DF_CHAIN_WG", false, "factorisation: workgroups of the chain role at most (default 32)"},
     {"DBAT_HIP_DF_L2", false, "factorisation: 1 = finished tiles of the compact layout are read through the L2", "0|1"},
     {"DBAT_HIP_COV_DENSE", false, "posterior covariance: the dense inverse of the reduced system (rocsolver_dpotri) instead of the selected inversion"},
diff --git a/dbat_amd/csrc/nd.hpp b/dbat_amd/csrc/nd.hpp
--- a/dbat_amd/csrc/nd.hpp
+++ b/dbat_amd/csrc/nd.hpp
@@ -1,6 +1,7 @@
 #pragma once
 #include <algorithm>
 #include <cstdint>
+#include <cstdlib>
 #include <functional>
 #include <vector>
 
@@ -12,22 +13,81 @@
     std::vector<int> block_end;
     std::vector<int> block_owner;
     std::vector<uint8_t> block_sep;
+    std::vector<int> block_first;
     std::vector<int> cam_owner;
     int n_top_cams = 0;
 };
 
+inline void nd_min_cover(const std::vector<int> &L, const std::vector<int> &R, const uint64_t *adj, int adj_words,
+                         std::vector<int> &ridx ,
+                         std::vector<uint8_t> &inL, std::vector<uint8_t> &inR) {
+    const int nl = (int)L.size(), nr = (int)R.size();
+    for (int r = 0; r < nr; ++r) ridx[R[r]] = r;
+    std::vector<int> ptr(nl + 1, 0), nb;
+    for (int l = 0; l < nl; ++l) {
+        const uint64_t *row = adj + (size_t)L[l] * adj_words;
+        for (int w = 0; w < adj_words; ++w) {
+            uint64_t m = row[w];
+            while (m) {
+                const int b = 64 * w + __builtin_ctzll(m);
+                m &= m - 1;
+                if (ridx[b] >= 0) nb.push_back(ridx[b]);
+            }
+        }
+        ptr[l + 1] = (int)nb.size();
+    }
+    for (int r = 0; r < nr; ++r) ridx[R[r]] = -1;
+    std::vector<int> matchL(nl, -1), matchR(nr, -1), seen(nr, -1), it(nl, 0), via(nl, -1), stack;
+    for (int l0 = 0; l0 < nl; ++l0) {
+        stack.assign(1, l0); it[l0] = ptr[l0];
+        while (!stack.empty()) {
+            const int l = stack.back();
+            if (it[l] == ptr[l + 1]) { stack.pop_back(); continue; }
+            const int r = nb[it[l]++];
+            if (seen[r] == l0) continue;
+            seen[r] = l0; via[l] = r;
+            if (matchR[r] < 0) {
+                for (int lq : stack) { matchL[lq] = via[lq]; matchR[via[lq]] = lq; }
+                break;
+            }
+            it[matchR[r]] = ptr[matchR[r]];
+            stack.push_back(matchR[r]);
+        }
+    }
+    std::vector<uint8_t> zl(nl, 0), zr(nr, 0);
+    stack.clear();
+    for (int l = 0; l < nl; ++l) if (matchL[l] < 0) { zl[l] = 1; stack.push_back(l); }
+    while (!stack.empty()) {
+        const int l = stack.back(); stack.pop_back();
+        for (int q = ptr[l]; q < ptr[l + 1]; ++q) {
+            const int r = nb[q];
+            if (zr[r]) continue;
+            zr[r] = 1;
+            const int l2 = matchR[r];
+            if (l2 >= 0 && !zl[l2]) { zl[l2] = 1; stack.push_back(l2); }
+        }
+    }
+    inL.assign(nl, 0); inR.assign(nr, 0);
+    for (int l = 0; l < nl; ++l) inL[l] = !zl[l];
+    for (int r = 0; r < nr; ++r) inR[r] = zr[r];
+}
+
 inline void nd_build(int nc, const uint64_t *adj, int adj_words, const double *xyz, const double *weight,
-                     int nparts, int leaf, bool nd_off, NdTree &T) {
+                     int nparts, int leaf, bool nd_off, int sep_mode, NdTree &T) {
     T = NdTree();
     T.nparts = std::max(1, nparts);
     T.order.reserve(nc);
     T.cam_owner.assign(nc, 0);
-    auto adjacent = [&](int a, int b) { return (adj[(size_t)a * adj_words + (b >> 6)] >> (b & 63)) & 1ull; };
-    auto emit = [&](std::vector<int> &cams, int owner, bool sep = false) {
+    auto emit = [&](std::vector<int> &cams, int owner, bool sep = false, int first = -1) {
         std::sort(cams.begin(), cams.end());
         for (int c : cams) { T.order.push_back(c); T.cam_owner[c] = owner; if (owner < 0) ++T.n_top_cams; }
-        if (!cams.empty()) { T.block_end.push_back((int)T.order.size()); T.block_owner.push_back(owner); T.block_sep.push_back(sep ? 1 : 0); }
+        if (!cams.empty()) {
+            T.block_first.push_back(first >= 0 ? first : (int)T.block_end.size());
+            T.block_end.push_back((int)T.order.size()); T.block_owner.push_back(owner); T.block_sep.push_back(sep ? 1 : 0);
+        }
     };
+    std::vector<uint64_t> maskA((size_t)adj_words), maskB((size_t)adj_words);
+    std::vector<int> ridx((size_t)nc, -1);
     std::function<void(std::vector<int> &, int, int)> nd = [&](std::vector<int> &cams, int part0, int np) {
         if (cams.empty()) return;
         if (np == 1 && (int)cams.size() <= leaf) { emit(cams, part0); return; }
@@ -39,14 +99,25 @@
         std::stable_sort(s.begin(), s.end(), [&](int a, int b) { return xyz[3 * a + ax] < xyz[3 * b + ax]; });
         size_t half = s.size() / 2;
         const int npa = np / 2, npb = np - npa;
-        std::vector<int> A, B, Sep, A2;
+        std::vector<int> A, B, Sep, A2, B2;
+        auto boundary = [&](const int *from, size_t n, const std::vector<uint64_t> &mask, std::vector<int> &touch, std::vector<int> &rest) {
+            touch.clear(); rest.clear();
+            for (size_t q = 0; q < n; ++q) {
+                const uint64_t *row = adj + (size_t)from[q] * adj_words;
+                uint64_t any = 0;
+                for (int w = 0; w < adj_words && !any; ++w) any = row[w] & mask[w];
+                (any ? touch : rest).push_back(from[q]);
+            }
+        };
+        auto set_masks = [&](size_t h) {
+            std::fill(maskA.begin(), maskA.end(), 0); std::fill(maskB.begin(), maskB.end(), 0);
+            for (size_t q = 0; q < h; ++q) maskA[s[q] >> 6] |= 1ull << (s[q] & 63);
+            for (size_t q = h; q < s.size(); ++q) maskB[s[q] >> 6] |= 1ull << (s[q] & 63);
+        };
         auto cut = [&](size_t h) {
-            A.assign(s.begin(), s.begin() + h); B.assign(s.begin() + h, s.end()); Sep.clear(); A2.clear();
-            for (int a : A) {
-                bool touch = false;
-                for (int b : B) if (adjacent(a, b)) { touch = true; break; }
-                (touch ? Sep : A2).push_back(a);
-            }
+            set_masks(h);
+            B.assign(s.begin() + h, s.end()); B2 = B;
+            boundary(s.data(), h, maskB, Sep, A2);
         };
         if (np > 1) {
             auto wsum = [&](const std::vector<int> &v) { double t = 0; for (int c : v) t += weight ? weight[c] : 1.0; return t; };
@@ -63,13 +134,47 @@
             half = std::min(std::max<size_t>(half, 1), s.size() - 1);
         }
         cut(half);
+        if (np == 1 && sep_mode > 0) {
+            const long n = (long)s.size();
+            const long slide[5] = {0, -(n / 40), n / 40, -(n / 20), n / 20};
+            const int npos = sep_mode >= 2 ? 5 : 1;
+            long best_key[3] = {0, 0, 0};
+            bool have = false;
+            std::vector<int> bA, bB, bS, La, Lb, Ia, Ib, cS, cA, cB;
+            std::vector<uint8_t> inL, inR;
+            auto offer = [&](const std::vector<int> &Sc, const std::vector<int> &Ac, const std::vector<int> &Bc) {
+                const long key[3] = {(6 * (long)Sc.size() + 63) / 64, (long)Sc.size(), std::labs((long)Ac.size() - (long)Bc.size())};
+                if (have && !std::lexicographical_compare(key, key + 3, best_key, best_key + 3)) return;
+                have = true; std::copy(key, key + 3, best_key);
+                bS = Sc; bA = Ac; bB = Bc;
+            };
+            for (int p = 0; p < npos; ++p) {
+                const long h = (long)half + slide[p];
+                if (h < 1 || h > n - 1 || (p > 0 && slide[p] == 0)) continue;
+                set_masks((size_t)h);
+                boundary(s.data(), (size_t)h, maskB, La, Ia);
+                boundary(s.data() + h, (size_t)(n - h), maskA, Lb, Ib);
+                cA.assign(s.begin(), s.begin() + h); cB.assign(s.begin() + h, s.end());
+                offer(La, Ia, cB);
+                offer(Lb, cA, Ib);
+                if (La.empty()) continue;
+                std::sort(La.begin(), La.end()); std::sort(Lb.begin(), Lb.end());
+                nd_min_cover(La, Lb, adj, adj_words, ridx, inL, inR);
+                cS.clear(); cA = Ia; cB = Ib;
+                for (size_t q = 0; q < La.size(); ++q) (inL[q] ? cS : cA).push_back(La[q]);
+                for (size_t q = 0; q < Lb.size(); ++q) (inR[q] ? cS : cB).push_back(Lb[q]);
+                offer(cS, cA, cB);
+            }
+            Sep.swap(bS); A2.swap(bA); B2.swap(bB);
+        }
         if (Sep.size() * 2 >= cams.size() || A2.empty()) {
             emit(cams, np > 1 ? -1 : part0);
             return;
         }
+        const int first = (int)T.block_end.size();
         nd(A2, part0, np > 1 ? npa : 1);
-        nd(B, np > 1 ? part0 + npa : part0, np > 1 ? npb : 1);
-        emit(Sep, np > 1 ? -1 : part0, true);
+        nd(B2, np > 1 ? part0 + npa : part0, np > 1 ? npb : 1);
+        emit(Sep, np > 1 ? -1 : part0, true, first);
     };
     std::vector<int> all(nc);
     for (int c = 0; c < nc; ++c) all[c] = c;
@@ -77,4 +182,71 @@
     else nd(all, 0, T.nparts);
 }
 
-}
+inline int nd_check(int nc, const uint64_t *adj, int adj_words, const NdTree &T) {
+    const int nb = (int)T.block_end.size();
+    if ((int)T.order.size() != nc || (int)T.block_first.size() != nb || (nb ? T.block_end[nb - 1] : 0) != nc) return 1;
+    std::vector<int> blk((size_t)nc, -1);
+    for (int b = 0, q = 0; b < nb; ++b) {
+        if (T.block_end[b] <= q) return 1;
+        for (; q < T.block_end[b]; ++q) {
+            const int c = T.order[q];
+            if (c < 0 || c >= nc || blk[c] >= 0) return 1;
+            blk[c] = b;
+        }
+    }
+    for (int b = 0; b < nb; ++b) {
+        const int f = T.block_first[b];
+        if (f < 0 || f > b) return 2;
+        for (int d = f; d < b; ++d) if (T.block_first[d] < f) return 2;
+    }
+    for (int a = 0; a < nc; ++a)
+        for (int w = 0; w < adj_words; ++w) {
+            uint64_t m = adj[(size_t)a * adj_words + w];
+            while (m) {
+                const int b = 64 * w + __builtin_ctzll(m);
+                m &= m - 1;
+                if (b >= nc || blk[b] <= blk[a]) continue;
+                if (T.block_first[blk[b]] > blk[a]) return 3;
+            }
+        }
+    return 0;
+}
+
+struct NdScore {
+    int mode = -1, cams = 0, blocks = 0, tile_cols = 0, tiles = 0, chain = 0, run = 0, model = 0, valid = -1;
+    long long products = 0;
+    double model_us = 0.0;
+};
+using NdScoreFn = void (*)(int nc, int nio, const uint64_t *adj, int adj_words, const NdTree &T, NdScore &sc);
+inline NdScoreFn &nd_score_hook() { static NdScoreFn f = nullptr; return f; }
+
+inline int nd_select(int nc, int nio, const uint64_t *adj, int adj_words, const double *xyz, const double *weight,
+                     int nparts, int leaf, bool nd_off, int forced, bool score_forced, NdTree &T, NdScore *sc) {
+    NdScore local[3];
+    if (!sc) sc = local;
+    for (int m = 0; m < 3; ++m) sc[m] = NdScore();
+    const NdScoreFn score = nd_score_hook();
+    auto run = [&](int m, NdTree &t) {
+        nd_build(nc, adj, adj_words, xyz, weight, nparts, leaf, nd_off, m, t);
+        if (score && (score_forced || forced < 0 || forced > 2)) { score(nc, nio, adj, adj_words, t, sc[m]); sc[m].mode = m; }
+    };
+    if ((forced >= 0 && forced <= 2) || !score || nd_off) {
+        const int m = forced >= 0 && forced <= 2 ? forced : 0;
+        run(m, T);
+        return m;
+    }
+    NdTree cand[3];
+    int best = 0;
+    for (int m = 0; m < 3; ++m) {
+        nd_build(nc, adj, adj_words, xyz, weight, nparts, leaf, nd_off, m, cand[m]);
+        int same = -1;
+        for (int q = 0; q < m && same < 0; ++q) if (cand[q].order == cand[m].order && cand[q].block_end == cand[m].block_end) same = q;
+        if (same >= 0) { sc[m] = sc[same]; sc[m].mode = m; continue; }
+        score(nc, nio, adj, adj_words, cand[m], sc[m]); sc[m].mode = m;
+        if (m > 0 && sc[m].chain <= sc[0].chain && sc[m].model_us < 0.99 * sc[0].model_us && sc[m].model_us < sc[best].model_us) best = m;
+    }
+    T = std::move(cand[best]);
+    return best;
+}
+
+}
diff --git a/dbat_amd/csrc/plan.hpp b/dbat_amd/csrc/plan.hpp
--- a/dbat_amd/csrc/plan.hpp
+++ b/dbat_amd/csrc/plan.hpp
@@ -102,6 +102,10 @@
     std::vector<uint64_t> cam_adj;
     int cam_adj_words = 0;
     NdTree nd;
+    int nd_sep = 0;
+    NdScore nd_score[3];
+    std::vector<double> nd_xyz, nd_weight;
+    int nd_leaf = 32;
     bool mg_subtree = false;
     int max_k = 0;
     bool shared_eo = false;
@@ -853,7 +857,17 @@
             wcam[c] = (double)n_cam[c];
         }
         const int leaf = std::max(8, env_int("DBAT_HIP_ND_LEAF", 32));
-        nd_build(nc, P.cam_adj.data(), P.cam_adj_words, xyz.data(), wcam.data(), P.mg_subtree ? P.nranks : 1, leaf, nd_off, P.nd);
+        const bool stats = env_on("DBAT_HIP_PLAN_STATS");
+        const int forced = permuted_ok ? env_int("DBAT_HIP_ND_SEP", -1) : 0;
+        P.nd_sep = nd_select(nc, P.nIOu, P.cam_adj.data(), P.cam_adj_words, xyz.data(), wcam.data(), P.mg_subtree ? P.nranks : 1, leaf, nd_off,
+                             forced, stats, P.nd, P.nd_score);
+        for (int m = 0; m < 3 && stats; ++m)
+            if (P.nd_score[m].mode == m)
+                fprintf(stderr, "[plan] separators %d (%s): %d tile columns, %d tiles, longest chain %d, %lld tile products, modelled %.0f us (%s)%s\n",
+                        m, m == 0 ? "lower boundary at the median" : m == 1 ? "minimum cover at the median" : "minimum cover, slid cuts",
+                        P.nd_score[m].tile_cols, P.nd_score[m].tiles, P.nd_score[m].chain, P.nd_score[m].products, P.nd_score[m].model_us,
+                        P.nd_score[m].model ? "chain / products estimate" : "list schedule", m == P.nd_sep ? (forced >= 0 && forced <= 2 ? "  <- DBAT_HIP_ND_SEP" : "  <- chosen") : "");
+        P.nd_xyz.swap(xyz); P.nd_weight.swap(wcam); P.nd_leaf = leaf;
     }
     lapt("nested dissection");
     P.CMAX = env_int("DBAT_HIP_CMAX", P.with_io ? Plan::SIG_IO_CMAX : 21);
```
